# malcolmgreaves/deequ

Measured on AMD Instinct MI355X. Metric: rows/sec (whole node) for fused 16-col profile scan; % of HBM peak BW, higher is better.
Workload: dtype f64+int64+utf8; 1 GPU; C5 fused 16-col profile scan (8 f64 + 4 i64 + 4 utf8, 10% nulls) + state merge + incremental StateLoader append; rows_per_gpu=1000000000, chunk_rows=125000000, analyzers=93, parallelism=row-shard x1

## Files before the change

### deequ_amd/_lib.py

```python
from __future__ import annotations

import ctypes
import os

ABI_VERSION = 6

_HERE = os.path.dirname(os.path.abspath(__file__))
LIB_PATH = os.environ.get("DQ_LIB_PATH") or os.path.join(_HERE, "libdqscan.so")

DQ_OK = 0
DQ_E_INVALID = -1
DQ_E_TYPE = -2
DQ_E_UNSUPPORTED = -3
DQ_E_HIP = -4
DQ_E_OOM = -5
DQ_E_STATE = -6

TYPE_F64, TYPE_I64, TYPE_I32, TYPE_UTF8, TYPE_LARGE_UTF8 = 1, 2, 3, 4, 5
TYPE_F32, TYPE_I16, TYPE_I8, TYPE_BOOL, TYPE_DATE32, TYPE_TIMESTAMP = 6, 7, 8, 9, 10, 11
TYPE_DECIMAL128 = 12


def decimal_type(precision: int, scale: int) -> int:
    if not (1 <= precision <= 38 and 0 <= scale <= precision):
        raise ValueError(f"DecimalType({precision},{scale}) is not a GPU column type (precision 1..38, scale 0..p)")
    return TYPE_DECIMAL128 | precision << 8 | scale << 16

VARIANT_NAMES = {0: "validity", 1: "f64_stats", 2: "f64_stats_hll", 3: "f64_hll", 4: "i64_stats",
                 5: "i64_stats_hll", 6: "i64_hll", 7: "i32_stats", 8: "i32_stats_hll", 9: "i32_hll",
                 10: "utf8_hll", 11: "large_utf8_hll", 12: "utf8_dtype", 13: "utf8_hll_dtype",
                 14: "large_utf8_dtype", 15: "large_utf8_hll_dtype", 16: "f64_dtype",
                 17: "f32_stats", 18: "f32_stats_hll", 19: "f32_hll", 20: "i16_stats", 21: "i16_stats_hll",
                 22: "i16_hll", 23: "i8_stats", 24: "i8_stats_hll", 25: "i8_hll", 26: "f32_dtype", 27: "bool",
                 28: "d128_stats", 29: "d128_stats_hll", 30: "d128_hll", 31: "d128_dtype"}

OP_SIZE = 1
OP_COMPLETENESS = 2
OP_COMPLIANCE = 3
OP_SUM = 4
OP_MEAN = 5
OP_STDDEV = 6
OP_MIN = 7
OP_MAX = 8
OP_CORRELATION = 9
OP_APPROX_COUNT_DISTINCT = 10
OP_DATATYPE = 11
OP_PATTERN_MATCH = 12

PRED_COLUMN = 1
PRED_LIT_INT = 2
PRED_LIT_DECIMAL = 3
PRED_LIT_DOUBLE = 4
PRED_LIT_NULL = 5
PRED_LIT_BOOL = 6
PRED_CMP = 7
PRED_AND = 8
PRED_OR = 9
PRED_NOT = 10
PRED_IS_NULL = 11
PRED_IS_NOT_NULL = 12
PRED_COALESCE = 13
PRED_REGEX = 14

REGEX_RLIKE = 0
REGEX_EXTRACT_NONEMPTY = 1
REGEX_FULL = 2

CMP_LT, CMP_LE, CMP_GT, CMP_GE, CMP_EQ, CMP_NE = 1, 2, 3, 4, 5, 6


class ColumnDesc(ctypes.Structure):
    _fields_ = [("type", ctypes.c_int32), ("nullable", ctypes.c_int32)]


class AnalyzerSpec(ctypes.Structure):
    _fields_ = [("op", ctypes.c_int32), ("col_a", ctypes.c_int32), ("col_b", ctypes.c_int32),
                ("pred_root", ctypes.c_int32), ("where_root", ctypes.c_int32)]


class PredNode(ctypes.Structure):
    _fields_ = [("kind", ctypes.c_int32), ("a", ctypes.c_int32), ("b", ctypes.c_int32),
                ("cmp", ctypes.c_int32), ("i64", ctypes.c_int64), ("f64", ctypes.c_double)]


PRED_PASS = {"auto": 0, "interpreter": 1, "compiled": 2}


class PlanOptions(ctypes.Structure):
    _fields_ = [("struct_size", ctypes.c_int32), ("pred_pass", ctypes.c_int32), ("reserved", ctypes.c_int32 * 6)]


class ColumnView(ctypes.Structure):
    _fields_ = [("values", ctypes.c_void_p), ("validity", ctypes.c_void_p), ("offsets", ctypes.c_void_p),
                ("reserved", ctypes.c_int64)]


class _Size(ctypes.Structure):
    _fields_ = [("num_matches", ctypes.c_int64)]


class _Ratio(ctypes.Structure):
    _fields_ = [("num_matches", ctypes.c_int64), ("count", ctypes.c_int64)]


class _Sum(ctypes.Structure):
    _fields_ = [("sum", ctypes.c_double), ("partial", ctypes.c_int64), ("partial_hi", ctypes.c_int64),
                ("guard", ctypes.c_double), ("dec_scale", ctypes.c_int32), ("dec_digits", ctypes.c_int32)]


class _Mean(ctypes.Structure):
    _fields_ = [("sum", ctypes.c_double), ("count", ctypes.c_int64), ("partial", ctypes.c_int64),
                ("partial_hi", ctypes.c_int64), ("guard", ctypes.c_double), ("dec_scale", ctypes.c_int32),
                ("dec_digits", ctypes.c_int32)]


class _StdDev(ctypes.Structure):
    _fields_ = [("n", ctypes.c_double), ("avg", ctypes.c_double), ("m2", ctypes.c_double)]


class _MinMax(ctypes.Structure):
    _fields_ = [("value", ctypes.c_double)]


class _Corr(ctypes.Structure):
    _fields_ = [("n", ctypes.c_double), ("x_avg", ctypes.c_double), ("y_avg", ctypes.c_double),
                ("ck", ctypes.c_double), ("x_mk", ctypes.c_double), ("y_mk", ctypes.c_double)]


class _Hll(ctypes.Structure):
    _fields_ = [("words", ctypes.c_int64 * 52)]


class _DType(ctypes.Structure):
    _fields_ = [("num_null", ctypes.c_int64), ("num_fractional", ctypes.c_int64), ("num_integral", ctypes.c_int64),
                ("num_boolean", ctypes.c_int64), ("num_string", ctypes.c_int64)]


class _StateUnion(ctypes.Union):
    _fields_ = [("size", _Size), ("ratio", _Ratio), ("sum", _Sum), ("mean", _Mean), ("stddev", _StdDev),
                ("minmax", _MinMax), ("corr", _Corr), ("hll", _Hll), ("dtype", _DType)]


class FreqSummary(ctypes.Structure):
    _fields_ = [("num_groups", ctypes.c_int64), ("num_unique", ctypes.c_int64), ("num_values", ctypes.c_int64),
                ("entropy", ctypes.c_double)]


class State(ctypes.Structure):
    _fields_ = [("op", ctypes.c_int32), ("has_value", ctypes.c_uint8 * 2), ("integral", ctypes.c_uint8),
                ("reserved", ctypes.c_uint8), ("u", _StateUnion)]


STATE_SIZE = ctypes.sizeof(State)


class DQError(RuntimeError):
    def __init__(self, status: int, message: str):
        super().__init__(f"dqscan error {status}: {message}")
        self.status = status
        self.message = message


def _load():
    if not os.path.exists(LIB_PATH):
        raise ImportError(
            f"{LIB_PATH} is missing: build it with `make -C deequ_amd` or __graft_entry__.build(); "
            "the MI355X scan has no CPU fallback")
    import torch
    L = ctypes.CDLL(LIB_PATH)
    c = ctypes
    P = c.POINTER
    L.dq_abi_version.restype = c.c_int32
    L.dq_last_error.restype = c.c_char_p
    L.dq_plan_create.restype = c.c_int32
    L.dq_plan_create.argtypes = [P(AnalyzerSpec), c.c_int32, P(ColumnDesc), c.c_int32, P(PredNode), c.c_int32,
                                 c.c_int32, P(c.c_void_p)]
    L.dq_plan_create_ex.restype = c.c_int32
    L.dq_plan_create_ex.argtypes = [P(AnalyzerSpec), c.c_int32, P(ColumnDesc), c.c_int32, P(PredNode), c.c_int32,
                                    P(c.c_char_p), c.c_int32, c.c_int32, P(c.c_void_p)]
    L.dq_plan_create_opts.restype = c.c_int32
    L.dq_plan_create_opts.argtypes = [P(AnalyzerSpec), c.c_int32, P(ColumnDesc), c.c_int32, P(PredNode), c.c_int32,
                                      P(c.c_char_p), c.c_int32, P(PlanOptions), c.c_int32, P(c.c_void_p)]
    L.dq_plan_explain.restype = c.c_int64
    L.dq_plan_explain.argtypes = [P(AnalyzerSpec), c.c_int32, P(ColumnDesc), c.c_int32, P(PredNode), c.c_int32,
                                  P(c.c_char_p), c.c_int32, P(PlanOptions), c.c_char_p, c.c_int64]
    L.dq_plan_create_time.restype = c.c_int32
    L.dq_plan_create_time.argtypes = [c.c_void_p, P(c.c_double), P(c.c_double)]
    L.dq_regex_info.restype = c.c_int32
    L.dq_regex_info.argtypes = [c.c_char_p, c.c_int32, P(c.c_int32), P(c.c_int32)]
    L.dq_pred_pool_create.restype = c.c_int32
    L.dq_pred_pool_create.argtypes = [P(c.c_char_p), P(c.c_int32), c.c_int32, P(c.c_void_p)]
    L.dq_pred_pool_add.restype = c.c_int32
    L.dq_pred_pool_add.argtypes = [c.c_void_p, c.c_char_p, P(c.c_int32)]
    L.dq_pred_pool_add_regex.restype = c.c_int32
    L.dq_pred_pool_add_regex.argtypes = [c.c_void_p, c.c_int32, c.c_char_p, c.c_int32, P(c.c_int32)]
    L.dq_pred_pool_size.restype = c.c_int32
    L.dq_pred_pool_size.argtypes = [c.c_void_p]
    L.dq_pred_pool_nodes.restype = P(PredNode)
    L.dq_pred_pool_nodes.argtypes = [c.c_void_p]
    L.dq_pred_pool_num_patterns.restype = c.c_int32
    L.dq_pred_pool_num_patterns.argtypes = [c.c_void_p]
    L.dq_pred_pool_patterns.restype = P(c.c_char_p)
    L.dq_pred_pool_patterns.argtypes = [c.c_void_p]
    L.dq_pred_pool_destroy.restype = None
    L.dq_pred_pool_destroy.argtypes = [c.c_void_p]
    L.dq_regex_match_host.restype = c.c_int32
    L.dq_regex_match_host.argtypes = [c.c_char_p, c.c_int32, c.c_void_p, c.c_void_p, c.c_int64, c.c_void_p]
    L.dq_freq_build.restype = c.c_int32
    L.dq_freq_build.argtypes = [P(c.c_int32), c.c_int32, P(ColumnView), P(c.c_int64), c.c_int32, c.c_int32,
                                c.c_void_p, P(c.c_void_p)]
    L.dq_freq_merge.restype = c.c_int32
    L.dq_freq_merge.argtypes = [c.c_void_p, c.c_void_p, P(c.c_void_p)]
    L.dq_freq_summarize.restype = c.c_int32
    L.dq_freq_summarize.argtypes = [c.c_void_p, c.c_int64, P(FreqSummary)]
    L.dq_freq_num_groups.restype = c.c_int64
    L.dq_freq_num_groups.argtypes = [c.c_void_p]
    L.dq_freq_export.restype = c.c_int32
    L.dq_freq_export.argtypes = [c.c_void_p, c.c_void_p, c.c_void_p, c.c_int64]
    L.dq_mutual_information.restype = c.c_int32
    L.dq_mutual_information.argtypes = [P(c.c_int32), P(ColumnView), P(c.c_int64), c.c_int32, c.c_int64, c.c_int32,
                                        c.c_void_p, P(c.c_double), P(c.c_int32)]
    L.dq_approx_quantiles.restype = c.c_int32
    L.dq_approx_quantiles.argtypes = [c.c_int32, P(ColumnView), P(c.c_int64), c.c_int32, P(c.c_double), c.c_int32,
                                      c.c_double, c.c_int32, c.c_void_p, P(c.c_double), P(c.c_int64)]
    L.dq_quantile_digest.restype = c.c_int32
    L.dq_quantile_digest.argtypes = [c.c_int32, P(ColumnView), P(c.c_int64), c.c_int32, c.c_double, c.c_int32,
                                     c.c_void_p, P(c.c_double), P(c.c_int64), c.c_int64, P(c.c_int64), P(c.c_int64)]
    L.dq_freq_top.restype = c.c_int32
    L.dq_freq_top.argtypes = [c.c_void_p, c.c_int32, P(c.c_uint64), P(c.c_int64), P(c.c_uint64), P(c.c_int32)]
    L.dq_freq_destroy.restype = None
    L.dq_freq_destroy.argtypes = [c.c_void_p]
    L.dq_plan_set_stream.restype = c.c_int32
    L.dq_plan_set_stream.argtypes = [c.c_void_p, c.c_void_p]
    L.dq_scan.restype = c.c_int32
    L.dq_scan.argtypes = [c.c_void_p, P(ColumnView), c.c_int64, c.c_int64]
    L.dq_finish.restype = c.c_int32
    L.dq_finish.argtypes = [c.c_void_p, P(State)]
    L.dq_plan_reset.restype = c.c_int32
    L.dq_plan_reset.argtypes = [c.c_void_p]
    L.dq_plan_destroy.restype = None
    L.dq_plan_destroy.argtypes = [c.c_void_p]
    L.dq_plan_bytes_per_row_x1000.restype = c.c_int64
    L.dq_plan_bytes_per_row_x1000.argtypes = [c.c_void_p]
    L.dq_plan_num_launches.restype = c.c_int32
    L.dq_plan_num_launches.argtypes = [c.c_void_p]
    L.dq_plan_enable_timing.restype = c.c_int32
    L.dq_plan_enable_timing.argtypes = [c.c_void_p, c.c_int32]
    L.dq_plan_kernel_time.restype = c.c_int32
    L.dq_plan_kernel_time.argtypes = [c.c_void_p, c.c_int32, P(c.c_double), P(c.c_int64)]
    L.dq_plan_variant_bytes_per_row_x1000.restype = c.c_int64
    L.dq_plan_variant_bytes_per_row_x1000.argtypes = [c.c_void_p, c.c_int32]
    L.dq_plan_kernel_bytes_per_row_x1000.restype = c.c_int64
    L.dq_plan_kernel_bytes_per_row_x1000.argtypes = [c.c_void_p, c.c_int32]
    L.dq_plan_pred_compiled.restype = c.c_int32
    L.dq_plan_pred_compiled.argtypes = [c.c_void_p, c.c_char_p, c.c_int32]
    L.dq_plan_pred_wait.restype = c.c_int32
    L.dq_plan_pred_wait.argtypes = [c.c_void_p, c.c_int32]
    L.dq_state_merge.restype = c.c_int32
    L.dq_state_merge.argtypes = [P(State), P(State), P(State)]
    L.dq_state_combine.restype = c.c_int32
    L.dq_state_combine.argtypes = [P(State), P(State), P(State)]
    for fn in ("dq_state_merge_n", "dq_state_combine_n"):
        getattr(L, fn).restype = c.c_int32
        getattr(L, fn).argtypes = [P(State), P(State), c.c_int32, P(State)]
    L.dq_state_is_defined.restype = c.c_int32
    L.dq_state_is_defined.argtypes = [P(State)]
    L.dq_state_metric.restype = c.c_int32
    L.dq_state_metric.argtypes = [P(State), P(c.c_double)]
    L.dq_hll_estimate.restype = c.c_int32
    L.dq_hll_estimate.argtypes = [P(c.c_int64), P(c.c_double)]
    L.dq_state_to_bytes.restype = c.c_int64
    L.dq_state_to_bytes.argtypes = [P(State), c.c_void_p, c.c_int64]
    L.dq_state_from_bytes.restype = c.c_int32
    L.dq_state_from_bytes.argtypes = [c.c_int32, c.c_char_p, c.c_int64, P(State)]
    L.dq_state_identifier.restype = c.c_int32
    L.dq_state_identifier.argtypes = [c.c_char_p]
    if L.dq_abi_version() != ABI_VERSION:
        raise ImportError(f"libdqscan ABI {L.dq_abi_version()} != {ABI_VERSION}")
    return L


lib = _load()

EXPORTED = [
    "dq_abi_version", "dq_last_error", "dq_plan_create", "dq_plan_create_ex", "dq_plan_create_opts",
    "dq_plan_create_time", "dq_plan_explain", "dq_regex_info", "dq_regex_match_host",
    "dq_pred_pool_create", "dq_pred_pool_add", "dq_pred_pool_add_regex", "dq_pred_pool_size", "dq_pred_pool_nodes",
    "dq_pred_pool_num_patterns", "dq_pred_pool_patterns", "dq_pred_pool_destroy",
    "dq_arrow_import", "dq_uploader_create", "dq_upload", "dq_upload_fence", "dq_upload_release", "dq_upload_sync",
    "dq_uploader_destroy",
    "dq_plan_set_stream", "dq_freq_build", "dq_freq_merge", "dq_freq_summarize", "dq_freq_num_groups",
    "dq_freq_export", "dq_freq_destroy", "dq_mutual_information", "dq_approx_quantiles", "dq_quantile_digest", "dq_freq_top", "dq_scan", "dq_finish",
    "dq_plan_reset", "dq_plan_destroy", "dq_plan_bytes_per_row_x1000", "dq_plan_num_launches",
    "dq_plan_enable_timing", "dq_plan_kernel_time", "dq_plan_variant_bytes_per_row_x1000",
    "dq_plan_kernel_bytes_per_row_x1000", "dq_plan_pred_compiled", "dq_plan_pred_wait",
    "dq_state_merge", "dq_state_combine", "dq_state_merge_n", "dq_state_combine_n", "dq_state_is_defined", "dq_state_metric", "dq_hll_estimate",
    "dq_state_to_bytes", "dq_state_from_bytes", "dq_state_identifier",
]


def check(status: int) -> None:
    if status != DQ_OK:
        raise DQError(status, lib.dq_last_error().decode("utf-8", "replace"))
```

### deequ_amd/csrc/dq_device.h

```cpp
#pragma once

#include <cstdint>

namespace dq {

constexpr int kBlock = 256;
constexpr int kWaves = kBlock / 64;
constexpr int kRowsPerLane = 8;
constexpr int kRowsPerIter = kBlock * kRowsPerLane;
constexpr int kMaxWG = 4096;
constexpr int kTargetWGs = 8192;
constexpr int kMaxCols = 64;
constexpr int kMaxColTasks = 256;
constexpr int kMaxSchemaCols = 1 << 16;
constexpr int kMaxWhere = 8;
constexpr int kHllCopies = 8;
constexpr int kPredAccCopies = 16;
constexpr int kMaxRoots = 32;
constexpr int kMaxCounters = 32;
constexpr int kMaxInstr = 96;
constexpr int kPredStack = 16;
constexpr int kMaxRegexWords = 32768;

enum ColKind : int32_t {
  CK_F64 = 1, CK_I64 = 2, CK_I32 = 3, CK_UTF8 = 4, CK_LUTF8 = 5,
  CK_F32 = 6, CK_I16 = 7, CK_I8 = 8, CK_BOOL = 9,
  CK_D128 = 10,
  CK_D128_LO = 11, CK_D128_HI = 12, CK_D128_LOU = 13,
};
constexpr bool ck_float(int k) { return k == CK_F64 || k == CK_F32; }
constexpr int ck_bytes(int k) {
  return k >= CK_D128 ? 16 : k == CK_F64 || k == CK_I64 ? 8 : k == CK_I32 || k == CK_F32 ? 4 : k == CK_I16 ? 2 : 1;
}

enum ColVariant : int32_t {
  CV_VALIDITY = 0,
  CV_F64_S = 1, CV_F64_SH = 2, CV_F64_H = 3,
  CV_I64_S = 4, CV_I64_SH = 5, CV_I64_H = 6,
  CV_I32_S = 7, CV_I32_SH = 8, CV_I32_H = 9,
  CV_UTF8_H = 10, CV_LUTF8_H = 11,
  CV_UTF8_D = 12, CV_UTF8_HD = 13, CV_LUTF8_D = 14, CV_LUTF8_HD = 15, CV_F64_D = 16,
  CV_F32_S = 17, CV_F32_SH = 18, CV_F32_H = 19,
  CV_I16_S = 20, CV_I16_SH = 21, CV_I16_H = 22,
  CV_I8_S = 23, CV_I8_SH = 24, CV_I8_H = 25,
  CV_F32_D = 26, CV_BOOL = 27,
  CV_D128_S = 28, CV_D128_SH = 29, CV_D128_H = 30, CV_D128_D = 31,
};
constexpr int kNumVariants = 32;

constexpr int kMaxFinRanges = 2 * kNumVariants + 1;
struct FinRanges {
  int32_t n;
  int32_t first[kMaxFinRanges], end[kMaxFinRanges], nr[kMaxFinRanges];
};

struct ColTask {
  int32_t variant;
  int32_t col;
  int32_t where;
  int32_t hll_slot;
  int32_t arg;
  int32_t pad[3];
};

struct PairTask {
  int32_t col_x, col_y;
  int32_t kind_x, kind_y;
  int32_t where;
  int32_t pad[3];
};

constexpr int kTileCols = 8;
constexpr int kTilePairs = 32;
struct PairGroup {
  int32_t ncols;
  int32_t npairs;
  int32_t first_pair;
  int32_t where;
  int32_t cols[kTileCols];
  int32_t kinds[kTileCols];
  int8_t pi[kTilePairs], pj[kTilePairs];
};

constexpr int kPairWaves = 2;
constexpr int kPairPos = 8;
constexpr int kPairSlots = 14;
constexpr int kPairMoments = 4;
constexpr int kPairSlotA[kPairSlots] = {0, 2, 4, 6, 0, 2, 4, 6, 0, 2, 4, 6, 0, 2};
constexpr int kPairSlotB[kPairSlots] = {1, 3, 5, 7, 2, 4, 6, 0, 3, 5, 7, 1, 4, 6};
struct PairWaveTask {
  int32_t where;
  uint32_t pair_mask;
  uint32_t mom_mask;
  uint32_t swap_mask;
  int32_t cols[kPairPos];
  int32_t kinds[kPairPos];
  int32_t pair_out[kPairSlots];
  int32_t mom_out[kPairMoments];
};
struct PairWG {
  PairWaveTask wave[kPairWaves];
};

struct alignas(16) ColPartial {
  double n, mean, m2;
  double sum;
  int64_t isum;
  int64_t count;
  int64_t nan_count;
  double fmin, fmax;
  int64_t pinf_count;
  int64_t ninf_count;
  int64_t isum_hi;
};
static_assert(sizeof(ColPartial) == 96, "ColPartial layout");

struct alignas(16) CorrPartial {
  double n, xa, ya, ck, xm, ym, pad0, pad1;
};
static_assert(sizeof(CorrPartial) == 64, "CorrPartial layout");

struct alignas(16) PredPartial {
  int64_t t[kMaxCounters];
  int64_t nn[kMaxCounters];
};

enum PredOp : int32_t {
  PO_ATOM_CMP = 1,
  PO_ATOM_ISNULL = 2,
  PO_ATOM_NOTNULL = 3,
  PO_CONST = 4,
  PO_AND = 5,
  PO_OR = 6,
  PO_NOT = 7,
  PO_STORE = 8,
  PO_ATOM_REGEX = 9,
};
enum CmpOp : int32_t { C_LT = 1, C_LE = 2, C_GT = 3, C_GE = 4, C_EQ = 5, C_NE = 6, C_FALSE = 7, C_TRUE = 8 };
enum CmpType : int32_t { CT_INT = 1, CT_DBL = 2 };
enum NullRes : int32_t { NR_FALSE = 0, NR_TRUE = 1, NR_NULL = 2 };

struct PredInstr {
  int32_t op;
  int32_t cmp;
  int32_t ctype;
  int32_t null_res;
  int32_t col_a;
  int32_t col_b;
  int32_t kind_a;
  int32_t kind_b;
  int64_t lit_i;
  double lit_d;
  int32_t slot;
  int32_t pad;
};

struct PredCounter {
  int32_t pred;
  int32_t where;
};

struct PredProgram {
  const uint16_t* regex;
  int32_t regex_words;
  int32_t n_instr;
  int32_t n_counters;
  int32_t n_bitmaps;
  int32_t n_loads;
  int32_t n_roots;
  int32_t stack_depth;
  int16_t load_instr[kMaxInstr];
  int32_t bitmap_root[kMaxWhere];
  PredCounter counters[kMaxCounters];
  PredInstr instr[kMaxInstr];
};

struct ScanCols {
  const void* values[kMaxCols];
  const uint32_t* validity[kMaxCols];
  const void* offsets[kMaxCols];
};

struct ScanBitmaps {
  uint64_t* where_bits[kMaxWhere];
  int64_t* rare_rows;
};

}
```

### deequ_amd/csrc/dq_kernels.hip

```cpp
#include <hip/hip_runtime.h>

#include <cstdint>
#include <type_traits>

#include "dq_device.h"
#include "dq_hash.h"
#include "dq_decimal.h"
#include "dq_lane.h"

namespace dq {

#define DQ_DEC_TABLE static __constant__ const
#include "dq_dec_tables.inc"
#undef DQ_DEC_TABLE
__device__ __forceinline__ DecTab dec_dev_tab() { return DecTab{kDecP10Lo, kDecP10Hi, kDecRcpHi, kDecRcpLo}; }

typedef uint32_t u32x4 __attribute__((ext_vector_type(4)));

__device__ __forceinline__ uint32_t ld32(const uint8_t* base, int64_t a) {
  return *reinterpret_cast<const uint32_t*>(base + a);
}
__device__ __forceinline__ uint32_t read4(const uint8_t* base, int64_t pos) {
  int64_t a = pos & ~int64_t(3);
  uint32_t sh = (uint32_t)(pos & 3) * 8u;
// ... 262 lines not shown
      const bool two = r + 32 < row1;
      if (validity) sel = ((uint64_t)(two ? ((const_u32s)validity)[w + 1] : 0u) << 32) | ((const_u32s)validity)[w];
      if (mask) sel &= ((uint64_t)(two ? ((const_u32s)mask)[w + 1] : 0u) << 32) | ((const_u32s)mask)[w];
      if (r + 64 > row1) sel &= (1ull << (row1 - r)) - 1ull;
    }
    if (sel == 0) continue;
    const double x = range_value<KIND>(vr, r - row0 + lane);
    const uint64_t fm = __builtin_amdgcn_ballot_w64(__builtin_isfinite(x)) & sel;
    if (fm != 0) return wave_uniform(wave_sum_f64(lane_bit(fm) ? x : 0.0) / (double)__builtin_popcountll(fm));
  }
  return 0.0;
}

template <bool INTEGRAL, bool MINMAX_SEP>
__device__ __forceinline__ void masked_moments(LaneMoments& a, double& lo, double& hi, double x, uint64_t b,
                                               double shift, uint64_t ma, uint64_t mb) {
  double d;
  uint64_t save;
  if constexpr (INTEGRAL) {
    asm volatile(
        "s_and_saveexec_b64 %[save], %[ma]\n\t"
        "v_add_f64 %[d], %[x], -%[sh]\n\t"
        "v_lshl_add_u64 %[is], %[b], 0, %[is]\n\t"
        "v_min_f64 %[lo], %[lo], %[x]\n\t"
        "v_max_f64 %[hi], %[hi], %[x]\n\t"
        "v_add_f64 %[sd], %[sd], %[d]\n\t"
        "v_fma_f64 %[sdd], %[d], %[d], %[sdd]\n\t"
        "s_mov_b64 exec, %[save]"
        : [sd] "+v"(a.sd), [sdd] "+v"(a.sdd), [is] "+v"(a.is), [lo] "+v"(lo), [hi] "+v"(hi), [d] "=&v"(d),
          [save] "=&s"(save)
        : [x] "v"(x), [sh] "s"(shift), [b] "v"(b), [ma] "s"(ma)
        : "scc");
  } else if constexpr (!MINMAX_SEP) {
    asm volatile(
        "s_and_saveexec_b64 %[save], %[ma]\n\t"
        "v_add_f64 %[d], %[x], -%[sh]\n\t"
        "v_min_f64 %[lo], %[lo], %[x]\n\t"
        "v_max_f64 %[hi], %[hi], %[x]\n\t"
        "v_add_f64 %[sd], %[sd], %[d]\n\t"
        "v_fma_f64 %[sdd], %[d], %[d], %[sdd]\n\t"
        "s_mov_b64 exec, %[save]"
        : [sd] "+v"(a.sd), [sdd] "+v"(a.sdd), [lo] "+v"(lo), [hi] "+v"(hi), [d] "=&v"(d), [save] "=&s"(save)
        : [x] "v"(x), [sh] "s"(shift), [ma] "s"(ma)
        : "scc");
  } else {
    asm volatile(
        "s_and_saveexec_b64 %[save], %[ma]\n\t"
        "v_add_f64 %[d], %[x], -%[sh]\n\t"
        "v_add_f64 %[sd], %[sd], %[d]\n\t"
        "v_fma_f64 %[sdd], %[d], %[d], %[sdd]\n\t"
        "s_and_b64 exec, %[save], %[mb]\n\t"
        "v_min_f64 %[lo], %[lo], %[x]\n\t"
        "v_max_f64 %[hi], %[hi], %[x]\n\t"
        "s_mov_b64 exec, %[save]"
        : [sd] "+v"(a.sd), [sdd] "+v"(a.sdd), [lo] "+v"(lo), [hi] "+v"(hi), [d] "=&v"(d), [save] "=&s"(save)
        : [x] "v"(x), [sh] "s"(shift), [ma] "s"(ma), [mb] "s"(mb)
        : "scc");
  }
}

template <int KIND, bool STATS, bool HLL>
__device__ __forceinline__ void numeric_block(const double (&x)[8], const uint64_t (&bits)[8], const uint64_t (&m)[8],
                                              double shift, ColStats& s, LaneMoments& a, int32_t* regs, int32_t& qmin) {
#pragma unroll
  for (int j = 0; j < 8; ++j) {
    if (STATS) masked_moments<!ck_float(KIND), false>(a, s.fmin, s.fmax, x[j], bits[j], shift, m[j], m[j]);
    if (HLL) {
      const HllKey key = ck_bytes(KIND) <= 4 ? hll_key_int((uint32_t)bits[j]) : hll_key_long(bits[j]);
      qmin = min(qmin, key.q);
      if (lane_bit(m[j])) atomicMax(reinterpret_cast<int32_t*>(reinterpret_cast<char*>(regs) + key.addr), key.q);
    }
  }
  if (HLL) {
    if (__builtin_amdgcn_ballot_w64(qmin < 0) != 0) {
#pragma unroll 1
      for (int j = 0; j < 8; ++j) {
        if (lane_bit(m[j])) hll_update(regs, ck_bytes(KIND) <= 4 ? xxh64_int((uint32_t)bits[j]) : xxh64_long(bits[j]));
      }
      qmin = 0;
    }
  }
}

template <int KIND, bool STATS, bool HLL>
__device__ __forceinline__ void float_block_checked(__amdgpu_buffer_rsrc_t vr, const uint32_t* validity,
                                                    const uint32_t* mask, int64_t base, int32_t rem, int32_t vo,
                                                    double shift, ColStats& s, LaneMoments& a, int32_t* regs,
                                                    int64_t& cnt_w, int64_t& nan_v, int64_t& pinf_v, int64_t& ninf_v) {
  constexpr bool kF32 = KIND == CK_F32;
  const int lane = threadIdx.x & 63;
#pragma unroll 1
  for (int j = 0; j < 8; ++j) {
    const int32_t left = rem - 64 * j;
    if (left <= 0) break;
    const int64_t r = base + 64 * j;
    uint64_t mj = ~0ull;
    {
      const int64_t w = r >> 5;
      const bool two = left > 32;
      if (validity) mj = ((uint64_t)(two ? ((const_u32s)validity)[w + 1] : 0u) << 32) | ((const_u32s)validity)[w];
      if (mask) mj &= ((uint64_t)(two ? ((const_u32s)mask)[w + 1] : 0u) << 32) | ((const_u32s)mask)[w];
      if (left < 64) mj &= (1ull << left) - 1ull;
    }
    uint64_t b;
    double xv;
    if constexpr (kF32) {
      b = __builtin_amdgcn_raw_buffer_load_b32(vr, vo + j * 256, 0, 2 );
      xv = (double)__builtin_bit_cast(float, (uint32_t)b);
    } else {
      const auto w2 = __builtin_amdgcn_raw_buffer_load_b64(vr, vo + j * 512, 0, 2 );
      b = ((uint64_t)w2[1] << 32) | w2[0];
      xv = __builtin_bit_cast(double, b);
    }
    const uint64_t nf = __builtin_amdgcn_ballot_w64(!__builtin_isfinite(xv)) & mj;
    const uint64_t nanm = __builtin_amdgcn_ballot_w64(xv != xv) & mj;
    const uint64_t inf = nf & ~nanm, pinf = __builtin_amdgcn_ballot_w64(xv > 0.0) & inf;
    if (lane == 0) {
      nan_v += __builtin_popcountll(nanm);
      pinf_v += __builtin_popcountll(pinf);
      ninf_v += __builtin_popcountll(inf & ~pinf);
    }
    if (STATS) {
      const uint64_t mm = mj & ~inf;
      cnt_w += __builtin_popcountll(mm);
      masked_moments<false, true>(a, s.fmin, s.fmax, xv, b, shift, mm, mj & ~nanm);
    } else {
      cnt_w += __builtin_popcountll(mj);
    }
    if (HLL) {
      if (lane_bit(nanm)) b = kF32 ? 0x7FC00000ull : 0x7FF8000000000000ull;
      const HllKey key = kF32 ? hll_key_int((uint32_t)b) : hll_key_long(b);
      if (lane_bit(mj)) {
        if (key.q >= 0) atomicMax(reinterpret_cast<int32_t*>(reinterpret_cast<char*>(regs) + key.addr), key.q);
        else hll_update(regs, kF32 ? xxh64_int((uint32_t)b) : xxh64_long(b));
      }
    }
  }
}

template <int K> struct KindT { using T = double; };
template <> struct KindT<CK_I64> { using T = int64_t; };
template <> struct KindT<CK_I32> { using T = int32_t; };
template <> struct KindT<CK_F32> { using T = float; };
template <> struct KindT<CK_I16> { using T = int16_t; };
template <> struct KindT<CK_I8> { using T = int8_t; };

template <int KIND, bool STATS, bool HLL>
__device__ void numeric_range(const void* values, const uint32_t* validity, const uint32_t* mask,
                              int64_t row0, int64_t row1, ColStats& s, int32_t* regs) {
  using T = typename KindT<KIND>::T;
  constexpr bool kLazy = ck_float(KIND) && STATS;
  const int lane = threadIdx.x & 63;
  const int wave = __builtin_amdgcn_readfirstlane(threadIdx.x >> 6);
  const T* v = reinterpret_cast<const T*>(values);
  const __amdgpu_buffer_rsrc_t vr = __builtin_amdgcn_make_buffer_rsrc(
      const_cast<T*>(v + row0), (short)0, (int)((row1 - row0) * (int64_t)sizeof(T)), 0x00020000);
  int64_t nan_v = 0, pinf_v = 0, ninf_v = 0;
  int64_t cnt_w = 0;
  LaneMoments a{0.0, 0.0, 0};
  const double shift = STATS ? range_shift_of<KIND>(vr, validity, mask, row0, row1, lane) : 0.0;
  int32_t qmin = 0;
  const int32_t nr = (int32_t)(row1 - row0);
  for (int32_t rb = 0; rb < nr; rb += kRowsPerIter) {
    const int64_t base = row0 + rb + wave * 512;
    const int32_t rem = nr - rb - wave * 512;
    const bool full = rb + kRowsPerIter <= nr;
    uint64_t bits[8], m[8];
    double x[8];
    const int32_t vo = (rb + wave * 512 + lane) * (int32_t)sizeof(T);
#pragma unroll
    for (int j = 0; j < 8; ++j) {
      if constexpr (sizeof(T) == 8) {
        const auto w2 = __builtin_amdgcn_raw_buffer_load_b64(vr, vo + j * 512, 0, 2 );
        bits[j] = ((uint64_t)w2[1] << 32) | w2[0];
        if (KIND == CK_F64) x[j] = __builtin_bit_cast(double, bits[j]);
        else x[j] = __builtin_fma((double)(int32_t)w2[1], 4294967296.0, (double)w2[0]);
      } else if constexpr (KIND == CK_F32) {
        const uint32_t w = __builtin_amdgcn_raw_buffer_load_b32(vr, vo + j * 256, 0, 2 );
        bits[j] = w;
        x[j] = (double)__builtin_bit_cast(float, w);
      } else {
        int32_t w;
        if constexpr (sizeof(T) == 4) w = (int32_t)__builtin_amdgcn_raw_buffer_load_b32(vr, vo + j * 256, 0, 2 );
        else if constexpr (sizeof(T) == 2) w = (int16_t)__builtin_amdgcn_raw_buffer_load_b16(vr, vo + j * 128, 0, 2 );
        else w = (int8_t)__builtin_amdgcn_raw_buffer_load_b8(vr, vo + j * 64, 0, 2 );
        bits[j] = (uint64_t)(int64_t)w;
        x[j] = (double)w;
      }
    }
    block_masks(validity, mask, base, rem, full, m);
    uint64_t nf_any = 0;
    if constexpr (ck_float(KIND) && !kLazy) {
#pragma unroll
      for (int j = 0; j < 8; ++j) nf_any |= __builtin_amdgcn_ballot_w64(!__builtin_isfinite(x[j])) & m[j];
    }
    if (ck_float(KIND) && !kLazy && nf_any != 0) {
      float_block_checked<KIND, STATS, HLL>(vr, validity, mask, base, rem, vo, shift, s, a, regs, cnt_w, nan_v, pinf_v,
                                            ninf_v);
    } else {
#pragma unroll
      for (int j = 0; j < 8; ++j) cnt_w += __builtin_popcountll(m[j]);
      numeric_block<KIND, STATS, HLL>(x, bits, m, shift, s, a, regs, qmin);
    }
  }
  if constexpr (kLazy) {
    __shared__ int32_t redo;
    if (threadIdx.x == 0) redo = 0;
    __syncthreads();
    const bool bad = !__builtin_isfinite(a.sd) || !__builtin_isfinite(a.sdd);
    if (__builtin_amdgcn_ballot_w64(bad) != 0 && lane == 0) redo = 1;
    __syncthreads();
    if (redo) {
      if (HLL) {
        for (int i = threadIdx.x; i < 512; i += kBlock) regs[i] = -1;
      }
      stats_init(s);
      a = LaneMoments{0.0, 0.0, 0};
      cnt_w = 0;
      __syncthreads();
      for (int32_t rb = 0; rb < nr; rb += kRowsPerIter) {
        const int32_t vo = (rb + wave * 512 + lane) * (int32_t)sizeof(T);
        float_block_checked<KIND, STATS, HLL>(vr, validity, mask, row0 + rb + wave * 512, nr - rb - wave * 512, vo,
                                              shift, s, a, regs, cnt_w, nan_v, pinf_v, ninf_v);
      }
    }
  }
  if (STATS) {
    const double S1 = wave_sum_f64(a.sd), S2 = wave_sum_f64(a.sdd);
    const int64_t is = ck_float(KIND) ? 0 : wave_sum_i64(a.is);
    if (lane == 0 && cnt_w > 0) {
      const double n = (double)cnt_w, q = S1 / n;
      s.n = n;
      s.mean = shift + q;
      const double m2 = __builtin_fma(-S1, q, S2);
      s.m2 = m2 < 0.0 ? 0.0 : m2;
      if (ck_float(KIND)) s.sum = __builtin_fma(n, shift, S1);
      else s.isum = is;
    }
  }
  if (lane == 0) s.count += cnt_w;
  if (ck_float(KIND) && lane == 0) {
    s.nan_count += nan_v;
    s.pinf += pinf_v;
    s.ninf += ninf_v;
    if (STATS) s.count += pinf_v + ninf_v;
  }
}

enum DtClass : uint32_t { DT_FRACTIONAL = 1, DT_INTEGRAL = 2, DT_BOOLEAN = 3, DT_STRING = 4 };

__device__ __forceinline__ uint32_t dt_class_of(bool numeric, uint32_t dots, bool boolean) {
  return numeric && dots <= 1 ? (dots ? DT_FRACTIONAL : DT_INTEGRAL) : (boolean ? DT_BOOLEAN : DT_STRING);
}

__device__ __forceinline__ uint32_t dt_keep(int lo, int hi) {
  const uint32_t below_hi = hi >= 4 ? 0x80808080u : (hi <= 0 ? 0u : 0x80808080u & ((1u << (8 * hi)) - 1u));
  const uint32_t from_lo = lo <= 0 ? 0x80808080u : (lo >= 4 ? 0u : 0x80808080u & ~((1u << (8 * lo)) - 1u));
  return below_hi & from_lo;
}

__device__ __forceinline__ uint32_t dt_class_short(const uint32_t (&w)[8], uint32_t len, bool active) {
  const uint32_t b0 = w[0] & 0xFFu;
  const uint32_t sgn = (len > 0 && (b0 == 0x2Bu || b0 == 0x2Du)) ? 1u : 0u;
  const uint32_t start = sgn + ((sgn < len && ((w[0] >> (8 * sgn)) & 0xFFu) == 0x20u) ? 1u : 0u);
  uint32_t bad = 0, dots = 0;
#pragma unroll
  for (int k = 0; k < 7; ++k) {
    if (k > 0 && __builtin_amdgcn_ballot_w64(active && bad == 0 && dots <= 1 && (uint32_t)(4 * k) < len) == 0) break;
    const uint32_t keep = dt_keep((int)start - 4 * k, (int)len - 4 * k);
    const uint32_t t = w[k] ^ 0x30303030u, z = w[k] ^ 0x2E2E2E2Eu;
    const uint32_t nd = ((t & 0x7F7F7F7Fu) + 0x76767676u) | t;
    const uint32_t nz = ((z & 0x7F7F7F7Fu) + 0x7F7F7F7Fu) | z;
    bad |= nd & nz & keep;
    dots += __builtin_popcount(~nz & keep);
  }
  const bool boolean = (len == 4 && w[0] == 0x65757274u) ||
                       (len == 5 && w[0] == 0x736C6166u && (w[1] & 0xFFu) == 0x65u);
  return dt_class_of(bad == 0, dots, boolean);
}

__device__ uint32_t dt_class_bytes(const uint8_t* p, int64_t len) {
  int64_t i = 0;
  if (len > 0 && (p[0] == '+' || p[0] == '-')) i = 1;
  if (i < len && p[i] == ' ') ++i;
  bool numeric = true;
  uint32_t dots = 0;
// ... 476 lines not shown
  const int32_t nr = (int32_t)(row1 - row0);
  for (int32_t rb = 0; rb < nr; rb += kRowsPerIter) {
    const int64_t base = row0 + rb + wave * 512;
    const int32_t rem = nr - rb - wave * 512;
    uint64_t m[8];
    block_masks(validity, mask, base, rem, rb + kRowsPerIter <= nr, m);
    uint64_t lo[8], hi[8];
#pragma unroll
    for (int j = 0; j < 8; ++j) load(base + 64 * j + lane, lo[j], hi[j]);
#pragma unroll
    for (int j = 0; j < 8; ++j) {
      cnt_w += __builtin_popcountll(m[j]);
      const bool sel = lane_bit(m[j]);
      if constexpr (STATS) {
        const double x = dec_to_double(lo[j], hi[j], sc, tab, prec <= 18);
        masked_moments<false, false>(a, s.fmin, s.fmax, x, 0, shift, m[j], m[j]);
        if (sel) {
          const uint64_t l2 = slo + lo[j];
          shi += hi[j] + (l2 < slo ? 1u : 0u);
          slo = l2;
          guard += x;
        }
      }
      if constexpr (HLL) {
        const uint64_t b = dec_hash_head(lo[j], hi[j], prec);
        const HllKey key = hll_key_from_fmix(b);
        if (sel) {
          if (key.q >= 0) atomicMax(reinterpret_cast<int32_t*>(reinterpret_cast<char*>(regs) + key.addr), key.q);
          else hll_update(regs, fmix_tail(b));
        }
      }
      if constexpr (DT) frac += __builtin_popcountll(__builtin_amdgcn_ballot_w64(dec_dt_class(lo[j], hi[j], sc, tab) == 1) & m[j]);
    }
  }
  if constexpr (STATS) {
    const double S1 = wave_sum_f64(a.sd), S2 = wave_sum_f64(a.sdd), G = wave_sum_f64(guard);
#pragma unroll
    for (int k = 32; k >= 1; k >>= 1) {
      const uint64_t olo = __shfl_xor(slo, k), ohi = __shfl_xor(shi, k);
      const uint64_t l2 = slo + olo;
      shi = shi + ohi + (l2 < slo ? 1u : 0u);
      slo = l2;
    }
    if (lane == 0 && cnt_w > 0) {
      const double n = (double)cnt_w, q = S1 / n;
      s.n = n;
      s.mean = shift + q;
      const double m2 = __builtin_fma(-S1, q, S2);
      s.m2 = m2 < 0.0 ? 0.0 : m2;
      s.sum = G;
      s.isum = (int64_t)slo;
      s.isum_hi = (int64_t)shi;
    }
  }
  if (lane == 0) {
    s.count += cnt_w;
    if (DT) s.isum += frac;
  }
}

__device__ void validity_range(const uint32_t* validity, const uint32_t* mask, int64_t row0, int64_t row1, ColStats& s) {
  const int64_t w0 = row0 >> 5, w1 = (row1 + 31) >> 5;
  int64_t c = 0;
  for (int64_t w = w0 + threadIdx.x; w < w1; w += kBlock) {
    uint32_t bits = word_or_ones(validity, w);
    if (mask) bits &= mask[w];
    const int64_t r = w << 5;
    if (r + 32 > row1) bits &= (1u << (row1 - r)) - 1u;
    c += __popc(bits);
  }
  s.count += c;
}

template <int KIND, bool STATS, bool HLL>
__device__ void run_numeric(const ColTask& t, const ScanCols& cols, const ScanBitmaps& bm, int64_t row0, int64_t row1,
                            ColStats& s, int32_t* regs) {
  const uint32_t* mask = t.where >= 0 ? reinterpret_cast<const uint32_t*>(bm.where_bits[t.where]) : nullptr;
  numeric_range<KIND, STATS, HLL>(cols.values[t.col], cols.validity[t.col], mask, row0, row1, s, regs);
}

template <int V, bool LONG>
__device__ __forceinline__ void run_variant(const ColTask& t, const ScanCols& cols, const uint32_t* mask, int64_t row0,
                                            int64_t row1, int64_t n_rows, ColStats& s, int32_t* regs,
                                            const uint64_t* p5, uint32_t* dq, uint32_t* rare, uint32_t* cls) {
  const void* v = cols.values[t.col];
  const uint32_t* val = cols.validity[t.col];
  if constexpr (V == CV_VALIDITY) validity_range(val, mask, row0, row1, s);
  else if constexpr (V == CV_F64_S) numeric_range<CK_F64, true, false>(v, val, mask, row0, row1, s, regs);
  else if constexpr (V == CV_F64_SH) numeric_range<CK_F64, true, true>(v, val, mask, row0, row1, s, regs);
  else if constexpr (V == CV_F64_H) numeric_range<CK_F64, false, true>(v, val, mask, row0, row1, s, regs);
  else if constexpr (V == CV_I64_S) numeric_range<CK_I64, true, false>(v, val, mask, row0, row1, s, regs);
  else if constexpr (V == CV_I64_SH) numeric_range<CK_I64, true, true>(v, val, mask, row0, row1, s, regs);
  else if constexpr (V == CV_I64_H) numeric_range<CK_I64, false, true>(v, val, mask, row0, row1, s, regs);
  else if constexpr (V == CV_I32_S) numeric_range<CK_I32, true, false>(v, val, mask, row0, row1, s, regs);
  else if constexpr (V == CV_I32_SH) numeric_range<CK_I32, true, true>(v, val, mask, row0, row1, s, regs);
  else if constexpr (V == CV_I32_H) numeric_range<CK_I32, false, true>(v, val, mask, row0, row1, s, regs);
  else if constexpr (V == CV_F32_S) numeric_range<CK_F32, true, false>(v, val, mask, row0, row1, s, regs);
  else if constexpr (V == CV_F32_SH) numeric_range<CK_F32, true, true>(v, val, mask, row0, row1, s, regs);
  else if constexpr (V == CV_F32_H) numeric_range<CK_F32, false, true>(v, val, mask, row0, row1, s, regs);
  else if constexpr (V == CV_I16_S) numeric_range<CK_I16, true, false>(v, val, mask, row0, row1, s, regs);
  else if constexpr (V == CV_I16_SH) numeric_range<CK_I16, true, true>(v, val, mask, row0, row1, s, regs);
  else if constexpr (V == CV_I16_H) numeric_range<CK_I16, false, true>(v, val, mask, row0, row1, s, regs);
  else if constexpr (V == CV_I8_S) numeric_range<CK_I8, true, false>(v, val, mask, row0, row1, s, regs);
  else if constexpr (V == CV_I8_SH) numeric_range<CK_I8, true, true>(v, val, mask, row0, row1, s, regs);
  else if constexpr (V == CV_I8_H) numeric_range<CK_I8, false, true>(v, val, mask, row0, row1, s, regs);
  else if constexpr (V == CV_F64_D) float_dtype_range(reinterpret_cast<const double*>(v), val, mask, row0, row1, s);
  else if constexpr (V == CV_F32_D) float_dtype_range(reinterpret_cast<const float*>(v), val, mask, row0, row1, s);
  else if constexpr (V == CV_BOOL) bool_range(reinterpret_cast<const uint32_t*>(v), val, mask, row0, row1, s, regs);
  else if constexpr (V == CV_D128_S) decimal_range<true, false, false>(v, val, mask, row0, row1, s, regs, t.arg);
  else if constexpr (V == CV_D128_SH) decimal_range<true, true, false>(v, val, mask, row0, row1, s, regs, t.arg);
  else if constexpr (V == CV_D128_H) decimal_range<false, true, false>(v, val, mask, row0, row1, s, regs, t.arg);
  else if constexpr (V == CV_D128_D) decimal_range<false, false, true>(v, val, mask, row0, row1, s, regs, t.arg);
  else if constexpr (V == CV_UTF8_H || V == CV_UTF8_D || V == CV_UTF8_HD)
    utf8_range<int32_t, V != CV_UTF8_D, V != CV_UTF8_H, LONG>(
        reinterpret_cast<const uint8_t*>(v), reinterpret_cast<const int32_t*>(cols.offsets[t.col]), val, mask, row0,
        row1, n_rows, s, regs, p5, dq, rare, cls);
  else
    utf8_range<int64_t, V != CV_LUTF8_D, V != CV_LUTF8_H, LONG>(
        reinterpret_cast<const uint8_t*>(v), reinterpret_cast<const int64_t*>(cols.offsets[t.col]), val, mask, row0,
        row1, n_rows, s, regs, p5, dq, rare, cls);
}

#ifndef DQ_STR_WAVES
#define DQ_STR_WAVES 6
#endif
#ifndef DQ_NUM_WAVES
#define DQ_NUM_WAVES 6
#endif
template <int V, bool LONG>
constexpr int kMinWaves = V == CV_UTF8_H && !LONG && DQ_STR_CLS ? 5
                          : V == CV_UTF8_H && DQ_STR_WAVES > 0 ? DQ_STR_WAVES
                          : (V == CV_F64_SH || V == CV_I64_SH) && DQ_NUM_WAVES > 0 ? DQ_NUM_WAVES
                          : V == CV_LUTF8_H && LONG ? 5
                                                    : 1;

template <int V, bool LONG = false>
__global__ __launch_bounds__(kBlock) __attribute__((amdgpu_waves_per_eu(kMinWaves<V, LONG>))) void dq_column_scan(const ColTask* __restrict__ tasks, int32_t ntasks,
                                                         int32_t part_base, ScanCols cols, ScanBitmaps bm,
                                                         int64_t n_rows, int64_t rows_per_range,
                                                         ColPartial* __restrict__ partials,
                                                         uint32_t* __restrict__ hll_acc) {
  constexpr bool kHll = !(V == CV_VALIDITY || V == CV_F64_S || V == CV_I64_S || V == CV_I32_S || V == CV_F64_D ||
                         V == CV_UTF8_D || V == CV_LUTF8_D || V == CV_F32_S || V == CV_I16_S || V == CV_I8_S ||
                         V == CV_F32_D || V == CV_BOOL || V == CV_D128_S || V == CV_D128_D);
  constexpr bool kBool = V == CV_BOOL;
  constexpr bool kStr = V == CV_UTF8_H || V == CV_LUTF8_H || V == CV_UTF8_HD || V == CV_LUTF8_HD;
  __shared__ int32_t regs[kHll ? 512 : 2];
  __shared__ uint64_t p5[kStr ? 256 : 1];
  constexpr uint32_t kDCap = DQ_STR_CLS && (V == CV_UTF8_H || V == CV_LUTF8_H) && !LONG ? kDefCapCls : kDefCap;
  __shared__ uint32_t dfq[kStr ? kWaves * kDefFields * kDCap : 1];
  __shared__ uint32_t rare[kStr ? kWaves : 1];
  constexpr bool kCls = DQ_STR_CLS && (V == CV_UTF8_H || V == CV_LUTF8_H) && !LONG;
  __shared__ __attribute__((aligned(16))) uint32_t clsbuf[kCls ? kWaves * kClsWords : 4];
  __shared__ ColStats red[kWaves];
  const int32_t ti = blockIdx.x % ntasks;
  const int32_t range = blockIdx.x / ntasks;
  const ColTask t = tasks[ti];
  const int64_t row0 = (int64_t)range * rows_per_range;
  int64_t row1 = row0 + rows_per_range;
  if (row1 > n_rows) row1 = n_rows;
  if constexpr (kBool) {
    if (threadIdx.x < 2) regs[threadIdx.x] = 0;
    __syncthreads();
  }
  if constexpr (kHll) {
    for (int i = threadIdx.x; i < 512; i += kBlock) regs[i] = -1;
    if constexpr (kStr) {
      p5[threadIdx.x] = (uint64_t)threadIdx.x * XP5;
      if (threadIdx.x < kWaves) rare[threadIdx.x] = 0;
    }
    __syncthreads();
  }
  ColStats s;
  stats_init(s);
  const uint32_t* mask = t.where >= 0 ? reinterpret_cast<const uint32_t*>(bm.where_bits[t.where]) : nullptr;
  const int32_t wv = kStr ? __builtin_amdgcn_readfirstlane(threadIdx.x >> 6) : 0;
  run_variant<V, LONG>(t, cols, mask, row0, row1, n_rows, s, regs, p5, dfq + wv * kDefFields * kDCap, rare + wv,
                       clsbuf + (kCls ? wv * kClsWords : 0));
  block_reduce_store(s, partials + (size_t)(part_base + ti) * kMaxWG + range, red);
  if constexpr (kStr) {
    if (threadIdx.x == 0 && bm.rare_rows) {
      uint32_t r = 0;
      for (int w = 0; w < kWaves; ++w) r += rare[w];
      if (r) atomicAdd(reinterpret_cast<unsigned long long*>(bm.rare_rows + part_base + ti), (unsigned long long)r);
    }
  }
  if constexpr (kBool) {
    if (threadIdx.x == 0 && t.hll_slot >= 0) {
      uint32_t* dst = hll_acc + ((size_t)t.hll_slot * kHllCopies + (blockIdx.x % kHllCopies)) * 512;
      for (int b = 0; b < 2; ++b) {
        if (!regs[b]) continue;
        const uint64_t x = xxh64_int(b == 0 ? 1u : 0u);
        atomicMax(dst + (uint32_t)(x >> 55), (uint32_t)(hll_q_exact(x) + 1));
      }
    }
  }
  if constexpr (kHll) {
    __syncthreads();
    uint32_t* dst = hll_acc + ((size_t)t.hll_slot * kHllCopies + (blockIdx.x % kHllCopies)) * 512;
    for (int i = threadIdx.x; i < 512; i += kBlock) {
      const uint32_t v = (uint32_t)(regs[i] + 1);
      if (v > __builtin_nontemporal_load(dst + i)) atomicMax(dst + i, v);
    }
  }
}

struct CorrStats { double n, xa, ya, ck, xm, ym; };

__device__ __forceinline__ void corr_merge(CorrStats& a, const CorrStats& b) {
  double n = a.n + b.n;
  if (b.n != 0.0) {
    if (a.n == 0.0) { a.xa = b.xa; a.ya = b.ya; a.ck = b.ck; a.xm = b.xm; a.ym = b.ym; }
    else {
      double dx = b.xa - a.xa, dy = b.ya - a.ya;
      double r = b.n / n;
      double dxr = dx * r, dyr = dy * r;
      a.ck = a.ck + b.ck + dx * dyr * a.n;
      a.xm = a.xm + b.xm + dx * dxr * a.n;
      a.ym = a.ym + b.ym + dy * dyr * a.n;
      a.xa = a.xa + dxr;
      a.ya = a.ya + dyr;
    }
  }
  a.n = n;
}

__device__ __forceinline__ int cmp_dbl(double a, double b) {
  bool an = a != a, bn = b != b;
  if (an || bn) return (an && bn) ? 0 : (an ? 1 : -1);
  return (a > b) - (a < b);
}
__device__ __forceinline__ bool apply_cmp(int op, int c) {
  switch (op) {
    case C_LT: return c < 0;
    case C_LE: return c <= 0;
    case C_GT: return c > 0;
    case C_GE: return c >= 0;
    case C_EQ: return c == 0;
    case C_NE: return c != 0;
    case C_TRUE: return true;
    default: return false;
  }
}

struct PredScratch {
  uint32_t *st, *sn, *rt, *rn, *ct, *cn;
  __device__ PredScratch(uint32_t* w, int depth, int roots, int counters) {
    st = w; sn = st + 16 * depth; rt = sn + 16 * depth; rn = rt + 16 * roots; ct = rn + 16 * roots; cn = ct + 16 * counters;
  }
};

__device__ __forceinline__ void pred_load(const void* p, int kind, int64_t row0, int64_t row1, int64_t base, int lane,
                                          uint64_t (&v)[8]) {
  if (kind == CK_BOOL) {
    const __amdgpu_buffer_rsrc_t r = __builtin_amdgcn_make_buffer_rsrc(
        const_cast<char*>(reinterpret_cast<const char*>(p) + (row0 >> 3)), (short)0, (int)(((row1 - row0 + 31) >> 5) * 4),
        0x00020000);
#pragma unroll
    for (int j = 0; j < 8; ++j) {
      const uint32_t w = __builtin_amdgcn_raw_buffer_load_b32(r, (int)(((base - row0) >> 5) + 2 * j + (lane >> 5)) * 4, 0, 0);
      v[j] = (w >> (lane & 31)) & 1u;
    }
    return;
  }
  const int sz = ck_bytes(kind);
  const __amdgpu_buffer_rsrc_t r = __builtin_amdgcn_make_buffer_rsrc(
      const_cast<char*>(reinterpret_cast<const char*>(p) + row0 * sz), (short)0, (int)((row1 - row0) * sz), 0x00020000);
  if (kind == CK_I32) {
#pragma unroll
    for (int j = 0; j < 8; ++j)
      v[j] = (uint64_t)(int64_t)(int32_t)__builtin_amdgcn_raw_buffer_load_b32(r, lane * 4, (int)((base - row0 + 64 * j) * 4), 2);
  } else if (kind == CK_F32) {
#pragma unroll
    for (int j = 0; j < 8; ++j)
      v[j] = __builtin_bit_cast(uint64_t, (double)__builtin_bit_cast(
                                              float, __builtin_amdgcn_raw_buffer_load_b32(r, (int)((base - row0 + 64 * j + lane) * 4), 0, 2)));
  } else if (kind == CK_I16) {
#pragma unroll
    for (int j = 0; j < 8; ++j)
      v[j] = (uint64_t)(int64_t)(int16_t)__builtin_amdgcn_raw_buffer_load_b16(r, (int)((base - row0 + 64 * j + lane) * 2), 0, 2);
  } else if (kind == CK_I8) {
#pragma unroll
    for (int j = 0; j < 8; ++j)
      v[j] = (uint64_t)(int64_t)(int8_t)__builtin_amdgcn_raw_buffer_load_b8(r, (int)(base - row0 + 64 * j + lane), 0, 2);
  } else if (kind >= CK_D128_LO) {
// ... 345 lines not shown
          for (int j = 0; j < 8; ++j) dst[j] = C.a[j];
        }
        vdst = C.va;
      } else if (same_blk && col == C.t_col_b && C.t_vals && (!vals || kind == C.t_kind_b)) {
        if (vals) {
#pragma unroll
          for (int j = 0; j < 8; ++j) dst[j] = C.b[j];
        }
        vdst = C.vb;
      } else {
        if (vals) pred_load(cols.values[col], kind, row0, row1, base, lane, dst);
        vdst = pred_valid_word(cols.validity[col], base, n_rows, lane);
      }
    };
    const bool cmp = op == PO_ATOM_CMP;
    if (cmp && col_b >= 0) fetch(col_b, kind_b, true, L.b, L.vb);
    fetch(col_a, kind_a, cmp, L.a, L.va);
    L.t_base = base;
    L.t_col_a = col_a;
    L.t_col_b = cmp ? col_b : -1;
    L.t_kind_a = kind_a;
    L.t_kind_b = kind_b;
    L.t_vals = cmp;
  };
  if (n_loads > 0) issue(0, row0 + (int64_t)wave * 512, B0, B1);
  uint32_t g = 0;

  for (int64_t blk = row0; blk < row1; blk += kRowsPerIter) {
    const int64_t base = blk + (int64_t)wave * 512;
    if (base >= row1) break;
    const int64_t wr = base + 32 * (lane & 15);
    const uint32_t inr = wr >= row1 ? 0u : (wr + 32 <= row1 ? ~0u : ((1u << (row1 - wr)) - 1u));
    int sp = 0, k = 0;
    for (int i = 0; i < n_instr; ++i) {
      const uint32_t ow = __builtin_amdgcn_readfirstlane(s_op[i]);
      const int op = (int)(ow & 0xFFu);
      if (op == PO_ATOM_CMP || op == PO_ATOM_ISNULL || op == PO_ATOM_NOTNULL || op == PO_ATOM_REGEX) {
        const int kn = k + 1 < n_loads ? k + 1 : 0;
        const int64_t bn = k + 1 < n_loads ? base : base + kRowsPerIter;
        uint32_t wt, wn;
        const AtomBuf& cur = (g & 1u) ? B1 : B0;
        if ((g & 1u) == 0) issue(kn, bn, B1, B0);
        else issue(kn, bn, B0, B1);
        if (op == PO_ATOM_CMP) {
          const PredInstr ins = uniform_cmp_fields(&s_instr[i]);
          if ((g & 1u) == 0) pred_atom_cmp(ins, B0, lane, wt, wn);
          else pred_atom_cmp(ins, B1, lane, wt, wn);
        } else if (RX && op == PO_ATOM_REGEX) {
          const PredInstr ins = uniform_instr(&s_instr[i]);
          const uint32_t va = (g & 1u) ? B1.va : B0.va;
          if (ins.kind_a == CK_UTF8)
            pred_atom_regex_utf8(ins, dfa_lds + ins.lit_i, reinterpret_cast<const uint8_t*>(cols.values[ins.col_a]),
                                 reinterpret_cast<const int32_t*>(cols.offsets[ins.col_a]), n_rows, row1, base, lane,
                                 va, wt, wn);
          else
            pred_atom_regex(ins, dfa_lds + ins.lit_i, reinterpret_cast<const uint8_t*>(cols.values[ins.col_a]),
                            cols.offsets[ins.col_a], row1, base, lane, va, wt, wn);
        } else {
          const uint32_t va = (g & 1u) ? B1.va : B0.va;
          wt = op == PO_ATOM_ISNULL ? ~va : va;
          wn = 0u;
        }
        (void)cur;
        ++g;
        ++k;
        if (wl) { S.st[(sp) * 16 + lane] = wt; S.sn[(sp) * 16 + lane] = wn; }
        ++sp;
      } else {
        pred_logic_op(ow, S, sp, lane);
      }
    }
    pred_block_out(S, s_ctr, n_counters, s_bmroot, n_bitmaps, bm, wr, inr, n_rows, lane);
  }
  pred_counters_out(pred_lds, wave_words, prog, acc);
}

__global__ __launch_bounds__(kBlock) void dq_finalize(int32_t ncol, int32_t nranges_col,
                                                      const ColPartial* __restrict__ col_part,
                                                      ColPartial* __restrict__ col_acc, int32_t npair, int32_t nranges_pair,
                                                      const CorrPartial* __restrict__ pair_part,
                                                      CorrPartial* __restrict__ pair_acc, int32_t has_pred,
                                                      int32_t nranges_pred, const PredPartial* __restrict__ pred_part,
                                                      PredPartial* __restrict__ pred_acc, FinRanges fr,
                                                      int64_t* __restrict__ rare_dev, int64_t* rare_host) {
  __shared__ ColStats cs[kBlock];
  __shared__ CorrStats ps[kBlock];
  const int b = blockIdx.x, tid = threadIdx.x;
  if (b < ncol) {
    int32_t nr = nranges_col;
    for (int i = 0; i < fr.n; ++i)
      if (b >= fr.first[i] && b < fr.end[i]) nr = fr.nr[i];
    ColStats s;
    stats_init(s);
    for (int r = tid; r < nr; r += kBlock) stats_merge(s, stats_load(col_part + (size_t)b * kMaxWG + r));
    cs[tid] = s;
    __syncthreads();
    for (int stride = kBlock / 2; stride >= 1; stride >>= 1) {
      if (tid < stride) { ColStats a = cs[tid]; stats_merge(a, cs[tid + stride]); cs[tid] = a; }
      __syncthreads();
    }
    if (tid == 0) {
      ColStats acc = stats_load(col_acc + b);
      stats_merge(acc, cs[0]);
      stats_store(col_acc + b, acc);
      if (rare_host && rare_dev[b] != rare_dev[ncol + b]) {
        rare_dev[ncol + b] = rare_dev[b];
        __hip_atomic_store(rare_host + b, rare_dev[b], __ATOMIC_RELAXED, __HIP_MEMORY_SCOPE_SYSTEM);
      }
    }
  } else if (b < ncol + npair) {
    const int p = b - ncol;
    CorrStats s = {0, 0, 0, 0, 0, 0};
    for (int r = tid; r < nranges_pair; r += kBlock) {
      const CorrPartial& q = pair_part[(size_t)p * kMaxWG + r];
      CorrStats o = {q.n, q.xa, q.ya, q.ck, q.xm, q.ym};
      corr_merge(s, o);
    }
    ps[tid] = s;
    __syncthreads();
    for (int stride = kBlock / 2; stride >= 1; stride >>= 1) {
      if (tid < stride) { CorrStats a = ps[tid]; corr_merge(a, ps[tid + stride]); ps[tid] = a; }
      __syncthreads();
    }
    if (tid == 0) {
      CorrPartial& q = pair_acc[p];
      CorrStats acc = {q.n, q.xa, q.ya, q.ck, q.xm, q.ym};
      corr_merge(acc, ps[0]);
      q.n = acc.n; q.xa = acc.xa; q.ya = acc.ya; q.ck = acc.ck; q.xm = acc.xm; q.ym = acc.ym;
    }
  } else if (has_pred) {
    static_assert(kBlock % kMaxCounters == 0, "counter layout");
    constexpr int G = kBlock / kMaxCounters;
    __shared__ int64_t st[G][kMaxCounters], sn[G][kMaxCounters];
    const int c = tid % kMaxCounters, g = tid / kMaxCounters;
    int64_t t = 0, nn = 0;
    for (int r = g; r < nranges_pred; r += G) { t += pred_part[r].t[c]; nn += pred_part[r].nn[c]; }
    st[g][c] = t;
    sn[g][c] = nn;
    __syncthreads();
    if (tid < kMaxCounters) {
      int64_t a = pred_acc->t[tid], b = pred_acc->nn[tid];
      for (int k = 0; k < G; ++k) { a += st[k][tid]; b += sn[k][tid]; }
      pred_acc->t[tid] = a;
      pred_acc->nn[tid] = b;
    }
  }
}

__global__ void dq_init_acc(ColPartial* col_acc, int32_t ncol, CorrPartial* pair_acc, int32_t npair, int64_t* rare_dev) {
  const int i = blockIdx.x * blockDim.x + threadIdx.x;
  if (i < ncol) {
    ColStats s;
    stats_init(s);
    stats_store(col_acc + i, s);
    if (rare_dev) rare_dev[i] = 0;
  }
  if (i < npair) {
    CorrPartial& q = pair_acc[i];
    q.n = q.xa = q.ya = q.ck = q.xm = q.ym = q.pad0 = q.pad1 = 0.0;
  }
}

hipError_t launch_pred_scan(const PredProgram* prog, const ScanCols& cols, const ScanBitmaps& bm, int64_t n_rows,
                            int64_t rows_per_range, int32_t nranges, PredPartial* acc, int32_t lds_bytes, hipStream_t st,
                            bool has_regex) {
  if (has_regex)
    hipLaunchKernelGGL(dq_pred_scan<true>, dim3(nranges), dim3(kBlock), (size_t)lds_bytes, st, prog, cols, bm, n_rows,
                       rows_per_range, acc);
  else
    hipLaunchKernelGGL(dq_pred_scan<false>, dim3(nranges), dim3(kBlock), (size_t)lds_bytes, st, prog, cols, bm, n_rows,
                       rows_per_range, acc);
  return hipGetLastError();
}

template <int V>
static void launch_v(const ColTask* tasks, int32_t ntasks, int32_t part_base, const ScanCols& cols,
                     const ScanBitmaps& bm, int64_t n_rows, int64_t rows_per_range, int32_t nranges,
                     ColPartial* partials, uint32_t* hll_acc, bool long_str, hipStream_t st) {
  constexpr bool kStrHll = V == CV_UTF8_H || V == CV_LUTF8_H || V == CV_UTF8_HD || V == CV_LUTF8_HD;
  if constexpr (kStrHll) {
    if (long_str) {
      hipLaunchKernelGGL((dq_column_scan<V, true>), dim3((uint32_t)ntasks * (uint32_t)nranges), dim3(kBlock), 0, st,
                         tasks, ntasks, part_base, cols, bm, n_rows, rows_per_range, partials, hll_acc);
      return;
    }
  }
  hipLaunchKernelGGL(dq_column_scan<V>, dim3((uint32_t)ntasks * (uint32_t)nranges), dim3(kBlock), 0, st, tasks, ntasks,
                     part_base, cols, bm, n_rows, rows_per_range, partials, hll_acc);
}

hipError_t launch_column_scan(int32_t variant, const ColTask* tasks, int32_t ntasks, int32_t part_base,
                              const ScanCols& cols, const ScanBitmaps& bm, int64_t n_rows, int64_t rows_per_range,
                              int32_t nranges, ColPartial* partials, uint32_t* hll_acc, bool long_str, hipStream_t st) {
#define DQ_V(V)                                                                                            \
  case V:                                                                                                  \
    launch_v<V>(tasks, ntasks, part_base, cols, bm, n_rows, rows_per_range, nranges, partials, hll_acc, long_str, \
                st);                                                                                       \
    break;
  switch (variant) {
    DQ_V(CV_VALIDITY) DQ_V(CV_F64_S) DQ_V(CV_F64_SH) DQ_V(CV_F64_H) DQ_V(CV_I64_S) DQ_V(CV_I64_SH) DQ_V(CV_I64_H)
    DQ_V(CV_I32_S) DQ_V(CV_I32_SH) DQ_V(CV_I32_H) DQ_V(CV_UTF8_H) DQ_V(CV_LUTF8_H)
    DQ_V(CV_UTF8_D) DQ_V(CV_UTF8_HD) DQ_V(CV_LUTF8_D) DQ_V(CV_LUTF8_HD) DQ_V(CV_F64_D)
    DQ_V(CV_F32_S) DQ_V(CV_F32_SH) DQ_V(CV_F32_H) DQ_V(CV_I16_S) DQ_V(CV_I16_SH) DQ_V(CV_I16_H)
    DQ_V(CV_I8_S) DQ_V(CV_I8_SH) DQ_V(CV_I8_H) DQ_V(CV_F32_D) DQ_V(CV_BOOL)
    DQ_V(CV_D128_S) DQ_V(CV_D128_SH) DQ_V(CV_D128_H) DQ_V(CV_D128_D)
    default: return hipErrorInvalidValue;
  }
#undef DQ_V
  return hipGetLastError();
}


hipError_t launch_finalize(int32_t ncol, int32_t nranges_col, const ColPartial* col_part, ColPartial* col_acc,
                           int32_t npair, int32_t nranges_pair, const CorrPartial* pair_part, CorrPartial* pair_acc,
                           int32_t has_pred, int32_t nranges_pred, const PredPartial* pred_part, PredPartial* pred_acc,
                           const FinRanges& fr, int64_t* rare_dev, int64_t* rare_host, hipStream_t st) {
  const uint32_t nb = (uint32_t)(ncol + npair + (has_pred ? 1 : 0));
  if (nb == 0) return hipSuccess;
  hipLaunchKernelGGL(dq_finalize, dim3(nb), dim3(kBlock), 0, st, ncol, nranges_col, col_part, col_acc, npair,
                     nranges_pair, pair_part, pair_acc, has_pred, nranges_pred, pred_part, pred_acc, fr, rare_dev,
                     rare_host);
  return hipGetLastError();
}

hipError_t launch_init_acc(ColPartial* col_acc, int32_t ncol, CorrPartial* pair_acc, int32_t npair, int64_t* rare_dev,
                           hipStream_t st) {
  const int n = ncol > npair ? ncol : npair;
  if (n == 0) return hipSuccess;
  hipLaunchKernelGGL(dq_init_acc, dim3((n + 255) / 256), dim3(256), 0, st, col_acc, ncol, pair_acc, npair, rare_dev);
  return hipGetLastError();
}

}
```

### deequ_amd/csrc/dq_plan.cpp

```cpp
#include <hip/hip_runtime.h>

#include <algorithm>
#include <chrono>
#include <cmath>
#include <cstdarg>
#include <cstdio>
#include <cstdlib>
#include <cstring>
#include <functional>
#include <iterator>
#include <limits>
#include <map>
#include <memory>
#include <string>
#include <tuple>
#include <vector>

#include "dq_device.h"
#include "dq_internal.h"
#include "dq_pred_jit.h"

#ifndef DQ_MIN_RANGE_ROWS
#define DQ_MIN_RANGE_ROWS 16384
#endif
#ifndef DQ_MIN_VALIDITY_RANGE_ROWS
#define DQ_MIN_VALIDITY_RANGE_ROWS 65536
#endif
#ifndef DQ_F64_HLL_DIV
#define DQ_F64_HLL_DIV 2
#endif
#ifndef DQ_PAIR_ONE_ROUND
#define DQ_PAIR_ONE_ROUND 1
#endif
#ifndef DQ_PRED_WGS
#define DQ_PRED_WGS 2048
#endif
#include "dq_regex.h"

namespace dq {

hipError_t launch_pred_scan(const PredProgram* prog, const ScanCols& cols, const ScanBitmaps& bm, int64_t n_rows,
                            int64_t rows_per_range, int32_t nranges, PredPartial* acc, int32_t lds_bytes, hipStream_t st,
                            bool has_regex);
hipError_t launch_column_scan(int32_t variant, const ColTask* tasks, int32_t ntasks, int32_t part_base,
                              const ScanCols& cols, const ScanBitmaps& bm, int64_t n_rows, int64_t rows_per_range,
                              int32_t nranges, ColPartial* partials, uint32_t* hll_acc, bool long_str, hipStream_t st);
hipError_t launch_pair_scan(const PairWG* wgs, int32_t nwg, const ScanCols& cols, const ScanBitmaps& bm,
                            const uint32_t* ones, int64_t n_rows, int64_t rows_per_range, int32_t nranges,
                            CorrPartial* pair_part, ColPartial* col_part, int32_t* redo, bool all_f64, bool ring,
                            bool minmax, hipStream_t st);
hipError_t pair_scan_residency(bool all_f64, bool ring, bool minmax, int32_t* per_cu);
hipError_t launch_finalize(int32_t ncol, int32_t nranges_col, const ColPartial* col_part, ColPartial* col_acc,
                           int32_t npair, int32_t nranges_pair, const CorrPartial* pair_part, CorrPartial* pair_acc,
                           int32_t has_pred, int32_t nranges_pred, const PredPartial* pred_part, PredPartial* pred_acc, const FinRanges& fr, int64_t* rare_dev, int64_t* rare_host,
                           hipStream_t st);
hipError_t launch_init_acc(ColPartial* col_acc, int32_t ncol, CorrPartial* pair_acc, int32_t npair, int64_t* rare_dev,
                           hipStream_t st);

static thread_local char g_err[1024] = "";
static thread_local bool g_capacity = false;

dq_status set_error(dq_status code, const char* fmt, ...) {
  va_list ap;
  va_start(ap, fmt);
  std::vsnprintf(g_err, sizeof(g_err), fmt, ap);
  va_end(ap);
  return code;
}

static dq_status cap_error(const char* fmt, ...) {
  va_list ap;
  va_start(ap, fmt);
  std::vsnprintf(g_err, sizeof(g_err), fmt, ap);
  va_end(ap);
  g_capacity = true;
  return DQ_E_UNSUPPORTED;
}

#define HIP_TRY(expr)                                                                              \
  do {                                                                                             \
    hipError_t e_ = (expr);                                                                        \
    if (e_ != hipSuccess)                                                                          \
      return set_error(e_ == hipErrorOutOfMemory ? DQ_E_OOM : DQ_E_HIP, "%s failed: %s (%s:%d)", \
                       #expr, hipGetErrorString(e_), __FILE__, __LINE__);                          \
  } while (0)

static bool is_numeric(int32_t t) {
  return t == DQ_TYPE_F64 || t == DQ_TYPE_I64 || t == DQ_TYPE_I32 || t == DQ_TYPE_F32 || t == DQ_TYPE_I16 ||
         t == DQ_TYPE_I8 || is_decimal(t);
}
static bool is_integral(int32_t t) { return t == DQ_TYPE_I64 || t == DQ_TYPE_I32 || t == DQ_TYPE_I16 || t == DQ_TYPE_I8; }
static bool is_floating(int32_t t) { return t == DQ_TYPE_F64 || t == DQ_TYPE_F32; }
static bool is_string(int32_t t) { return t == DQ_TYPE_UTF8 || t == DQ_TYPE_LARGE_UTF8; }
static int32_t kind_of(int32_t t) {
  switch (t) {
    case DQ_TYPE_F64: return CK_F64;
    case DQ_TYPE_I64: case DQ_TYPE_TIMESTAMP: return CK_I64;
    case DQ_TYPE_I32: case DQ_TYPE_DATE32: return CK_I32;
    case DQ_TYPE_F32: return CK_F32;
    case DQ_TYPE_I16: return CK_I16;
    case DQ_TYPE_I8: return CK_I8;
    case DQ_TYPE_BOOL: return CK_BOOL;
    case DQ_TYPE_UTF8: return CK_UTF8;
    case DQ_TYPE_LARGE_UTF8: return CK_LUTF8;
    default: return CK_D128;
  }
}
static int32_t pair_kind(int32_t t) {
  if (!is_decimal(t)) return kind_of(t);
  return CK_D128 | DQ_DECIMAL_SCALE(t) << 8 | (DQ_DECIMAL_PRECISION(t) <= 18 ? 1 : 0) << 16;
}
static int64_t value_bytes_x1000(int32_t t) {
  switch (t) {
    case DQ_TYPE_I32: case DQ_TYPE_F32: case DQ_TYPE_DATE32: case DQ_TYPE_UTF8: return 4000;
    case DQ_TYPE_I16: return 2000;
    case DQ_TYPE_I8: return 1000;
    case DQ_TYPE_BOOL: return 125;
    default: return is_decimal(t) ? 16000 : 8000;
  }
}
static double int_as_float(int64_t v) { return (double)(float)v; }

struct SpecOut {
  int32_t op = 0;
  int32_t col_task = -1;
  int32_t pair_task = -1;
  int32_t ctr_a = -1;
  int32_t ctr_b = -1;
  int32_t col_type = 0;
  bool has_where = false;
};

struct Lit {
  enum K { INT, DEC, DBL, NUL, BOOL } k;
  int64_t i = 0;
  int32_t scale = 0;
  double d = 0.0;
};

// ... 401 lines not shown
          return set_error(DQ_E_UNSUPPORTED, "float column compared with an int / long column");
        PredInstr p{};
        p.op = PO_ATOM_CMP; p.col_a = ca; p.col_b = cb; p.kind_a = kind_of(ta); p.kind_b = kind_of(tb);
        p.null_res = NR_NULL; p.cmp = to_cmpop(cmp);
        p.ctype = bools || (is_integral(ta) && is_integral(tb)) ? CT_INT : CT_DBL;
        out.push_back(p);
        return DQ_OK;
      }
      default:
        return set_error(DQ_E_UNSUPPORTED, "predicate node kind %d is not a boolean expression", n.kind);
    }
  }
};

static std::string canon(const dq_pred_node* pool, int32_t n_pred, int32_t idx, int depth = 0) {
  if (idx < 0 || idx >= n_pred || depth > 64) return "?";
  const dq_pred_node& n = pool[idx];
  char buf[128];
  std::snprintf(buf, sizeof(buf), "(%d:%d:%lld:%a", n.kind, n.cmp, (long long)n.i64, n.f64);
  std::string s = buf;
  if (n.kind == DQ_PRED_COLUMN) s += ":c" + std::to_string(n.a);
  else {
    if (n.kind == DQ_PRED_CMP || n.kind == DQ_PRED_AND || n.kind == DQ_PRED_OR || n.kind == DQ_PRED_NOT ||
        n.kind == DQ_PRED_IS_NULL || n.kind == DQ_PRED_IS_NOT_NULL || n.kind == DQ_PRED_COALESCE ||
        n.kind == DQ_PRED_REGEX)
      s += canon(pool, n_pred, n.a, depth + 1);
    if (n.kind == DQ_PRED_CMP || n.kind == DQ_PRED_AND || n.kind == DQ_PRED_OR || n.kind == DQ_PRED_COALESCE)
      s += canon(pool, n_pred, n.b, depth + 1);
  }
  return s + ")";
}

}

using namespace dq;

struct dq_plan {
  int32_t device = 0;
  hipStream_t stream = nullptr;
  bool own_stream = false;
  std::vector<dq_column_desc> schema;
  std::vector<dq_analyzer_spec> specs;
  std::vector<SpecOut> outs;

  std::vector<ColTask> col_tasks;
  struct Group { int32_t variant, first, count; };
  std::vector<Group> groups;
  std::vector<Group> pred_fused_groups;
  std::vector<PairTask> pair_tasks;
  std::vector<PairWG> pair_wgs;
  int32_t n_fused = 0;
  bool pair_all_f64 = true;
  bool pair_minmax = false;
  PredProgram prog{};
  std::vector<std::string> patterns;
  std::vector<uint16_t> regex_blob;
  uint16_t* d_regex = nullptr;
  int32_t n_hll = 0;
  bool has_pred = false;
  hipFunction_t pred_jit = nullptr;
  PredJitRef pred_jit_ref;
  std::vector<int32_t> pred_jit_cols;
  std::vector<int32_t> pred_jit_hll_task, pred_jit_hll_slot;
  int32_t pred_fused_first = 0, pred_fused_count = 0;
  int32_t pair_fused_first = 0, pair_fused_count = 0;
  int32_t pair_resident[2] = {0, 0};
  std::string pred_jit_note;
  int32_t pred_pass = DQ_PRED_PASS_AUTO;
  bool host_only = false;
  bool probe = false;
  std::string pred_jit_src;
  double create_ms = 0.0, pred_jit_ms = 0.0;

  ColTask* d_col_tasks = nullptr;
  PairTask* d_pair_tasks = nullptr;
  PairWG* d_pair_wgs = nullptr;
  int32_t* d_pair_redo = nullptr;
  char* h_stage = nullptr;
  int64_t* d_rare_dev = nullptr;
  int64_t* h_rare = nullptr;
  int64_t* d_rare = nullptr;
  std::vector<uint8_t> str_long;
  int32_t str_path = 0;
  int64_t prev_rows = 0;
  size_t h_stage_bytes = 0;
  PredProgram* d_prog = nullptr;
  ColPartial* d_col_part = nullptr;
  CorrPartial* d_pair_part = nullptr;
  PredPartial* d_pred_part = nullptr;
  ColPartial* d_col_acc = nullptr;
  uint32_t* d_hll_acc = nullptr;
  CorrPartial* d_pair_acc = nullptr;
  PredPartial* d_pred_acc = nullptr;
  uint64_t* d_where_bits[kMaxWhere] = {nullptr};
  int64_t where_cap_words = 0;
  uint32_t* d_ones = nullptr;
  int64_t ones_cap_words = 0;

  int64_t total_rows = 0;
  int64_t next_chunk = 0;

  bool timing = false;
  std::vector<hipEvent_t> ev_pool;
  struct Pending { int kernel; hipEvent_t a, b; };
  std::vector<Pending> pending;
  static constexpr int kTimers = 16 + kNumVariants;
  double kernel_ms[kTimers] = {0};
  int64_t kernel_launches[kTimers] = {0};
  int64_t bytes_per_row_x1000 = 0;
  int64_t pred_bytes_x1000 = 0, pair_bytes_x1000 = 0;
  int32_t launches_per_scan = 0;

  std::vector<dq_plan*> parts;
  std::vector<std::vector<int32_t>> part_specs;
  std::vector<std::vector<int32_t>> part_cols;
};

static dq_status take_event(dq_plan* p, hipEvent_t* e) {
  if (!p->ev_pool.empty()) { *e = p->ev_pool.back(); p->ev_pool.pop_back(); return DQ_OK; }
  HIP_TRY(hipEventCreate(e));
  return DQ_OK;
}

static dq_status resolve_timing(dq_plan* p) {
  if (p->pending.empty()) return DQ_OK;
  HIP_TRY(hipStreamSynchronize(p->stream));
  for (auto& q : p->pending) {
    float ms = 0.f;
    HIP_TRY(hipEventElapsedTime(&ms, q.a, q.b));
    p->kernel_ms[q.kernel] += ms;
    p->kernel_launches[q.kernel] += 1;
    p->ev_pool.push_back(q.a);
    p->ev_pool.push_back(q.b);
  }
  p->pending.clear();
  return DQ_OK;
}

template <typename F>
static dq_status timed(dq_plan* p, int kernel, hipStream_t st, F fn) {
  hipEvent_t a = nullptr, b = nullptr;
  if (p->timing) {
    if (dq_status s = take_event(p, &a)) return s;
    if (dq_status s = take_event(p, &b)) return s;
    HIP_TRY(hipEventRecord(a, st));
  }
  HIP_TRY(fn());
  if (p->timing) {
    HIP_TRY(hipEventRecord(b, st));
    p->pending.push_back({kernel, a, b});
  }
  return DQ_OK;
}

static dq_status free_plan_mem(dq_plan* p) {
  for (auto& q : p->pending) { p->ev_pool.push_back(q.a); p->ev_pool.push_back(q.b); }
  p->pending.clear();
  for (hipEvent_t e : p->ev_pool) (void)hipEventDestroy(e);
  p->ev_pool.clear();
  void* ptrs[] = {p->d_col_tasks, p->d_pair_tasks, p->d_pair_wgs, p->d_prog, p->d_col_part, p->d_pair_part,
                  p->d_pred_part, p->d_col_acc, p->d_hll_acc, p->d_pair_acc, p->d_pred_acc, p->d_regex, p->d_pair_redo,
                  p->d_rare_dev};
  for (void* q : ptrs)
    if (q) (void)hipFree(q);
  for (int i = 0; i < kMaxWhere; ++i)
    if (p->d_where_bits[i]) (void)hipFree(p->d_where_bits[i]);
  if (p->d_ones) (void)hipFree(p->d_ones);
  if (p->h_rare) (void)hipHostFree(p->h_rare);
  p->h_rare = p->d_rare = nullptr;
  if (p->h_stage) (void)hipHostFree(p->h_stage);
  p->h_stage = nullptr;
  p->h_stage_bytes = 0;
  return DQ_OK;
}

static dq_status reset_acc(dq_plan* p) {
  HIP_TRY(launch_init_acc(p->d_col_acc, (int32_t)p->col_tasks.size(), p->d_pair_acc, (int32_t)p->pair_tasks.size(),
                          p->d_rare_dev, p->stream));
  if (p->n_hll) HIP_TRY(hipMemsetAsync(p->d_hll_acc, 0, (size_t)p->n_hll * kHllCopies * 512 * sizeof(uint32_t), p->stream));
  if (p->has_pred) HIP_TRY(hipMemsetAsync(p->d_pred_acc, 0, kPredAccCopies * sizeof(PredPartial), p->stream));
  if (p->total_rows > 0) p->prev_rows = p->total_rows;
  p->total_rows = 0;
  p->next_chunk = 0;
  return DQ_OK;
}

template <typename T>
static dq_status dmalloc(T** ptr, size_t bytes) {
  if (bytes == 0) bytes = 16;
  HIP_TRY(hipMalloc((void**)ptr, bytes));
  return DQ_OK;
}

static void plan_pair_wgs(const dq_plan* p, const PairGroup& g, std::vector<PairWG>& out, std::vector<int>& fused) {
  auto blank = [&](const int32_t* lcols, int nl) {
    PairWG wg;
    std::memset(&wg, 0, sizeof(wg));
    for (int w = 0; w < kPairWaves; ++w) {
      PairWaveTask& t = wg.wave[w];
      t.where = g.where;
      for (int q = 0; q < kPairPos; ++q) {
        const int l = (q + w) % kPairPos;
        const int c = lcols[l < nl ? l : 0];
        t.cols[q] = g.cols[c];
        t.kinds[q] = g.kinds[c];
      }
      for (int q = 0; q < kPairSlots; ++q) t.pair_out[q] = -1;
      for (int k = 0; k < kPairMoments; ++k) t.mom_out[k] = -1;
    }
    return wg;
  };
  auto place = [&](PairWG& wg, int a, int b, int32_t pair) {
    for (int w = 0; w < kPairWaves; ++w) {
      const int pa = (a - w + kPairPos) % kPairPos, pb = (b - w + kPairPos) % kPairPos;
      for (int q = 0; q < kPairSlots; ++q) {
        const bool fwd = kPairSlotA[q] == pa && kPairSlotB[q] == pb, rev = kPairSlotA[q] == pb && kPairSlotB[q] == pa;
        if (!fwd && !rev) continue;
        PairWaveTask& t = wg.wave[w];
        if ((t.pair_mask >> q) & 1u) return false;
        t.pair_mask |= 1u << q;
        if (rev) t.swap_mask |= 1u << q;
        t.pair_out[q] = pair;
        return true;
      }
    }
    return false;
  };
  int32_t ident[kPairPos];
  for (int c = 0; c < kPairPos; ++c) ident[c] = c;
  PairWG wg = blank(ident, g.ncols);
  std::vector<int> extra;
  for (int q = 0; q < g.npairs; ++q)
    if (g.pi[q] == g.pj[q] || !place(wg, g.pi[q], g.pj[q], g.first_pair + q)) extra.push_back(q);
  for (int c = 0; c < g.ncols; ++c)
    for (size_t t = 0; t < p->col_tasks.size(); ++t) {
      const ColTask& ct = p->col_tasks[t];
      if (ct.col == g.cols[c] && ct.where == g.where && !fused[t] &&
          (ct.variant == CV_F64_S || ct.variant == CV_I64_S || ct.variant == CV_I32_S || ct.variant == CV_F32_S ||
           ct.variant == CV_I16_S || ct.variant == CV_I8_S)) {
        PairWaveTask& w = wg.wave[c % 2];
        const int k = (c - c % 2) / 2;
        w.mom_mask |= 1u << k;
        w.mom_out[k] = (int32_t)t;
        fused[t] = 1;
        break;
      }
    }
  if (wg.wave[0].pair_mask | wg.wave[0].mom_mask | wg.wave[1].pair_mask | wg.wave[1].mom_mask) out.push_back(wg);
  for (int q : extra) {
    const int32_t lc[2] = {g.pi[q], g.pj[q]};
    PairWG e = blank(lc, 2);
    PairWaveTask& t = e.wave[0];
    t.pair_mask = 1u;
    t.pair_out[0] = g.first_pair + q;
    out.push_back(e);
  }
}

static dq_status build_plan(dq_plan* p, const dq_pred_node* pool, int32_t n_pred) {
  const int32_t ncols = (int32_t)p->schema.size();
  std::map<std::string, int32_t> root_slot;
// ... 384 lines not shown
      p->pred_fused_groups.back().count++;
    }
    p->n_fused = (int32_t)std::count_if(fused.begin(), fused.end(), [](int f) { return f != 0; });
  }

  std::vector<int> need_values(ncols, 0), need_validity(ncols, 0);
  for (const ColTask& ct : p->col_tasks) {
    need_validity[ct.col] = 1;
    if (ct.variant != CV_VALIDITY) need_values[ct.col] = 1;
  }
  for (const PairTask& pt : p->pair_tasks) {
    need_values[pt.col_x] = need_values[pt.col_y] = 1;
    need_validity[pt.col_x] = need_validity[pt.col_y] = 1;
  }
  for (int i = 0; i < prog.n_instr; ++i) {
    const PredInstr& ins = prog.instr[i];
    if (ins.col_a >= 0) {
      need_validity[ins.col_a] = 1;
      if (ins.op == PO_ATOM_CMP || ins.op == PO_ATOM_REGEX) need_values[ins.col_a] = 1;
    }
    if (ins.col_b >= 0) { need_validity[ins.col_b] = 1; need_values[ins.col_b] = 1; }
  }
  int64_t b1000 = 0;
  for (int c = 0; c < ncols; ++c) {
    int32_t t = p->schema[c].type;
    if (need_values[c]) b1000 += value_bytes_x1000(t);
    if (need_validity[c] && p->schema[c].nullable) b1000 += 125;
  }
  p->bytes_per_row_x1000 = b1000;
  {
    auto bytes_of = [&](const std::vector<int>& vals, const std::vector<int>& valid) {
      int64_t b = 0;
      for (int c = 0; c < ncols; ++c) {
        int32_t t = p->schema[c].type;
        if (vals[c]) b += value_bytes_x1000(t);
        if (valid[c] && p->schema[c].nullable) b += 125;
      }
      return b;
    };
    std::vector<int> pv(ncols, 0), pn(ncols, 0), qv(ncols, 0), qn(ncols, 0);
    for (int i = 0; i < prog.n_instr; ++i) {
      const PredInstr& ins = prog.instr[i];
      if (ins.col_a >= 0) { pn[ins.col_a] = 1; if (ins.op == PO_ATOM_CMP || ins.op == PO_ATOM_REGEX) pv[ins.col_a] = 1; }
      if (ins.col_b >= 0) { pn[ins.col_b] = 1; pv[ins.col_b] = 1; }
    }
    for (const PairTask& pt : p->pair_tasks) { qv[pt.col_x] = qv[pt.col_y] = qn[pt.col_x] = qn[pt.col_y] = 1; }
    p->pred_bytes_x1000 = bytes_of(pv, pn);
    p->pair_bytes_x1000 = bytes_of(qv, qn);
  }
  p->launches_per_scan = (p->has_pred ? 1 : 0) + (int32_t)p->groups.size() + (p->pair_wgs.empty() ? 0 : 1) +
                         ((p->col_tasks.size() + p->pair_tasks.size()) ? 1 : 0);

  if (p->host_only) return DQ_OK;

  const size_t nct = p->col_tasks.size(), npt = p->pair_tasks.size();
  if (dq_status s = dmalloc(&p->d_col_tasks, nct * sizeof(ColTask))) return s;
  if (dq_status s = dmalloc(&p->d_pair_tasks, npt * sizeof(PairTask))) return s;
  if (dq_status s = dmalloc(&p->d_pair_wgs, p->pair_wgs.size() * sizeof(PairWG))) return s;
  if (!p->pair_wgs.empty())
    HIP_TRY(hipMemcpyAsync(p->d_pair_wgs, p->pair_wgs.data(), p->pair_wgs.size() * sizeof(PairWG),
                           hipMemcpyHostToDevice, p->stream));
  if (dq_status s = dmalloc(&p->d_pair_redo, p->pair_wgs.size() * kPairWaves * kMaxWG * sizeof(int32_t))) return s;
  if (dq_status s = dmalloc(&p->d_prog, sizeof(PredProgram))) return s;
  if (dq_status s = dmalloc(&p->d_col_part, nct * kMaxWG * sizeof(ColPartial))) return s;
  if (dq_status s = dmalloc(&p->d_pair_part, npt * kMaxWG * sizeof(CorrPartial))) return s;
  if (dq_status s = dmalloc(&p->d_pred_part, sizeof(PredPartial))) return s;
  if (dq_status s = dmalloc(&p->d_col_acc, nct * sizeof(ColPartial))) return s;
  if (dq_status s = dmalloc(&p->d_rare_dev, 2 * nct * sizeof(int64_t))) return s;
  if (nct) HIP_TRY(hipMemsetAsync(p->d_rare_dev, 0, 2 * nct * sizeof(int64_t), p->stream));
  p->str_long.assign(nct, 0);
  if (const char* e = std::getenv("DQ_STR_PATH")) p->str_path = std::strcmp(e, "fast") == 0 ? 1 : std::strcmp(e, "long") == 0 ? 2 : 0;
  if (nct && hipHostMalloc(reinterpret_cast<void**>(&p->h_rare), nct * sizeof(int64_t), hipHostMallocMapped) == hipSuccess) {
    std::memset(p->h_rare, 0, nct * sizeof(int64_t));
    void* dp = nullptr;
    if (hipHostGetDevicePointer(&dp, p->h_rare, 0) == hipSuccess) {
      p->d_rare = static_cast<int64_t*>(dp);
    } else {
      (void)hipHostFree(p->h_rare);
      p->h_rare = nullptr;
    }
  }
  (void)hipGetLastError();
  if (dq_status s = dmalloc(&p->d_hll_acc, (size_t)p->n_hll * kHllCopies * 512 * sizeof(uint32_t))) return s;
  if (dq_status s = dmalloc(&p->d_pair_acc, npt * sizeof(CorrPartial))) return s;
  if (dq_status s = dmalloc(&p->d_pred_acc, kPredAccCopies * sizeof(PredPartial))) return s;
  if (nct) HIP_TRY(hipMemcpyAsync(p->d_col_tasks, p->col_tasks.data(), nct * sizeof(ColTask), hipMemcpyHostToDevice, p->stream));
  if (npt) HIP_TRY(hipMemcpyAsync(p->d_pair_tasks, p->pair_tasks.data(), npt * sizeof(PairTask), hipMemcpyHostToDevice, p->stream));
  if (!p->regex_blob.empty()) {
    if (dq_status s = dmalloc(&p->d_regex, p->regex_blob.size() * sizeof(uint16_t))) return s;
    HIP_TRY(hipMemcpyAsync(p->d_regex, p->regex_blob.data(), p->regex_blob.size() * sizeof(uint16_t),
                           hipMemcpyHostToDevice, p->stream));
  }
  p->prog.regex = p->d_regex;
  p->prog.regex_words = (int32_t)p->regex_blob.size();
  HIP_TRY(hipMemcpyAsync(p->d_prog, &p->prog, sizeof(PredProgram), hipMemcpyHostToDevice, p->stream));
  if (dq_status s = reset_acc(p)) return s;
  HIP_TRY(hipStreamSynchronize(p->stream));
  return DQ_OK;
}



static void pred_columns(const dq_pred_node* pool, int32_t n_pred, int32_t idx, std::vector<int32_t>& cols,
                         int depth = 0) {
  if (idx < 0 || idx >= n_pred || depth > 64) return;
  const dq_pred_node& n = pool[idx];
  switch (n.kind) {
    case DQ_PRED_COLUMN: cols.push_back(n.a); return;
    case DQ_PRED_CMP: case DQ_PRED_AND: case DQ_PRED_OR: case DQ_PRED_COALESCE:
      pred_columns(pool, n_pred, n.a, cols, depth + 1);
      pred_columns(pool, n_pred, n.b, cols, depth + 1);
      return;
    case DQ_PRED_NOT: case DQ_PRED_IS_NULL: case DQ_PRED_IS_NOT_NULL: case DQ_PRED_REGEX:
      pred_columns(pool, n_pred, n.a, cols, depth + 1);
      return;
    default: return;
  }
}

static std::vector<int32_t> spec_columns(const dq_analyzer_spec& s, const dq_pred_node* pool, int32_t n_pred,
                                         int32_t ncols) {
  std::vector<int32_t> c;
  if (s.op == DQ_OP_CORRELATION) { c.push_back(s.col_a); c.push_back(s.col_b); }
  else if (s.op != DQ_OP_SIZE && s.op != DQ_OP_COMPLIANCE) c.push_back(s.col_a);
  pred_columns(pool, n_pred, s.pred_root, c);
  pred_columns(pool, n_pred, s.where_root, c);
  c.erase(std::remove_if(c.begin(), c.end(), [&](int32_t x) { return x < 0 || x >= ncols; }), c.end());
  std::sort(c.begin(), c.end());
  c.erase(std::unique(c.begin(), c.end()), c.end());
  return c;
}

struct PartInput {
  std::vector<dq_analyzer_spec> specs;
  std::vector<dq_column_desc> schema;
  std::vector<dq_pred_node> pool;
};

static void make_part_input(const std::vector<dq_analyzer_spec>& specs, const std::vector<dq_column_desc>& schema,
                            const dq_pred_node* pool, int32_t n_pred, const std::vector<int32_t>& spec_idx,
                            const std::vector<int32_t>& cols, PartInput& in) {
  const int32_t ncols = (int32_t)schema.size();
  std::vector<int32_t> local(ncols, -1);
  in.schema.clear();
  for (size_t j = 0; j < cols.size(); ++j) {
    local[cols[j]] = (int32_t)j;
    in.schema.push_back(schema[cols[j]]);
  }
  auto map = [&](int32_t c) { return c >= 0 && c < ncols ? local[c] : -1; };
  in.specs.clear();
  for (int32_t i : spec_idx) {
    dq_analyzer_spec sp = specs[i];
    if (sp.col_a >= 0) sp.col_a = map(sp.col_a);
    if (sp.col_b >= 0) sp.col_b = map(sp.col_b);
    in.specs.push_back(sp);
  }
  in.pool.assign(pool, pool + n_pred);
  for (dq_pred_node& n : in.pool)
    if (n.kind == DQ_PRED_COLUMN) n.a = map(n.a);
}

static dq_status plan_part_host(const dq_plan& parent, const dq_pred_node* pool, int32_t n_pred,
                                const std::vector<int32_t>& spec_idx, const std::vector<int32_t>& cols, bool probe,
                                dq_plan& q) {
  PartInput in;
  make_part_input(parent.specs, parent.schema, pool, n_pred, spec_idx, cols, in);
// ... 247 lines not shown

static dq_status check_view(const dq_column_desc& cd, const dq_column_view& v, int32_t c, int64_t n_rows) {
  const int32_t t = cd.type;
  if (v.reserved != 0) return set_error(DQ_E_INVALID, "dq_scan: column %d reserved field must be 0", c);
  if (n_rows > 0 && !v.values) return set_error(DQ_E_INVALID, "dq_scan: column %d has no values buffer", c);
  if (((uintptr_t)v.values & 15) != 0)
    return set_error(DQ_E_INVALID, "dq_scan: column %d values buffer must be 16-byte aligned", c);
  if (((uintptr_t)v.validity & 3) != 0)
    return set_error(DQ_E_INVALID, "dq_scan: column %d validity bitmap must be 4-byte aligned", c);
  if ((t == DQ_TYPE_UTF8 || t == DQ_TYPE_LARGE_UTF8) && n_rows > 0 && !v.offsets)
    return set_error(DQ_E_INVALID, "dq_scan: UTF8 column %d has no offsets", c);
  return DQ_OK;
}

extern "C" {

dq_status dq_scan(dq_plan* p, const dq_column_view* cols, int64_t n_rows, int64_t chunk_index) {
  if (!p) return set_error(DQ_E_INVALID, "dq_scan: plan is NULL");
  if (n_rows < 0) return set_error(DQ_E_INVALID, "dq_scan: n_rows < 0");
  if (n_rows >= (int64_t(1) << 31))
    return set_error(DQ_E_INVALID, "dq_scan: a chunk holds at most 2^31 - 1 rows (split larger inputs into chunks)");
  if (chunk_index != p->next_chunk)
    return set_error(DQ_E_INVALID, "dq_scan: chunk_index %lld out of order (expected %lld)", (long long)chunk_index,
                     (long long)p->next_chunk);
  const int32_t ncols = (int32_t)p->schema.size();
  if (ncols > 0 && !cols) return set_error(DQ_E_INVALID, "dq_scan: cols is NULL");
  HIP_TRY(hipSetDevice(p->device));
  if (!p->parts.empty()) {
    for (size_t k = 0; k < p->parts.size(); ++k) {
      for (int32_t c : p->part_cols[k])
        if (dq_status s = check_view(p->schema[c], cols[c], c, n_rows)) return s;
      if (p->parts[k]->next_chunk != chunk_index)
        return set_error(DQ_E_INVALID, "dq_scan: part %zu is at chunk %lld (expected %lld)", k,
                         (long long)p->parts[k]->next_chunk, (long long)chunk_index);
    }
    std::vector<dq_column_view> v;
    for (size_t k = 0; k < p->parts.size(); ++k) {
      v.resize(p->part_cols[k].size());
      for (size_t j = 0; j < v.size(); ++j) v[j] = cols[p->part_cols[k][j]];
      if (dq_status s = dq_scan(p->parts[k], v.data(), n_rows, chunk_index)) return s;
    }
    p->next_chunk++;
    p->total_rows += n_rows;
    return DQ_OK;
  }
  ScanCols sc{};
  for (int32_t c = 0; c < ncols; ++c)
    if (dq_status s = check_view(p->schema[c], cols[c], c, n_rows)) return s;
  for (int32_t c = 0; c < ncols; ++c) {
    const dq_column_view& v = cols[c];
    sc.values[c] = v.values;
    sc.validity[c] = p->schema[c].nullable ? reinterpret_cast<const uint32_t*>(v.validity) : nullptr;
    sc.offsets[c] = v.offsets;
  }
  p->next_chunk++;
  if (n_rows == 0) return DQ_OK;
  if (p->pred_jit_ref) {
    std::string note;
    if (hipFunction_t fn = pred_jit_poll(p->pred_jit_ref, 0, note)) {
      p->pred_jit = fn;
      p->pred_jit_note = note + " (compiled in the background; used from chunk " + std::to_string(chunk_index) + ")";
      p->pred_jit_ref.reset();
    } else if (!pred_jit_pending(p->pred_jit_ref)) {
      p->pred_jit_note = note;
      p->pred_jit_ref.reset();
    }
  }
  std::vector<dq_plan::Group> groups(p->groups);
  if (!p->pred_jit) groups.insert(groups.end(), p->pred_fused_groups.begin(), p->pred_fused_groups.end());

  const int64_t words = ceil_div(n_rows, 64);
  if (p->prog.n_bitmaps > 0 && words > p->where_cap_words) {
    HIP_TRY(hipStreamSynchronize(p->stream));
    for (int b = 0; b < p->prog.n_bitmaps; ++b) {
      if (p->d_where_bits[b]) (void)hipFree(p->d_where_bits[b]);
      p->d_where_bits[b] = nullptr;
      if (dq_status s = dmalloc(&p->d_where_bits[b], (size_t)words * 8 + 64)) return s;
    }
    p->where_cap_words = words;
  }
  ScanBitmaps bm{};
  for (int b = 0; b < kMaxWhere; ++b) bm.where_bits[b] = p->d_where_bits[b];
  bm.rare_rows = p->d_rare_dev;
  if ((!p->pair_wgs.empty() || p->pred_jit) && words + 1 > p->ones_cap_words) {
    HIP_TRY(hipStreamSynchronize(p->stream));
    if (p->d_ones) (void)hipFree(p->d_ones);
    p->d_ones = nullptr;
    if (dq_status s = dmalloc(&p->d_ones, (size_t)(words + 1) * 8)) return s;
    HIP_TRY(hipMemsetAsync(p->d_ones, 0xFF, (size_t)(words + 1) * 8, p->stream));
    p->ones_cap_words = words + 1;
  }

  int64_t min_launch = 0;
  for (const auto& g : groups) min_launch = min_launch ? std::min<int64_t>(min_launch, g.count) : g.count;
  if (!p->pair_wgs.empty()) {
    const int64_t wg = (int64_t)p->pair_wgs.size();
    min_launch = min_launch ? std::min<int64_t>(min_launch, wg) : wg;
  }
  const int64_t want = std::max<int64_t>(64, std::min<int64_t>(kMaxWG, kTargetWGs / std::max<int64_t>(1, min_launch)));
  auto size_ranges = [&](int64_t w, int64_t& rpr, int32_t& nr, int64_t min_rows) {
    w = std::min<int64_t>(w, std::max<int64_t>(1, n_rows / min_rows));
    nr = (int32_t)std::min<int64_t>(w, ceil_div(n_rows, kRowsPerIter));
    rpr = ceil_div(ceil_div(n_rows, nr), kRowsPerIter) * kRowsPerIter;
    nr = (int32_t)ceil_div(n_rows, rpr);
  };
  int32_t nr_col;
  int64_t rpr_col;
  size_ranges(want, rpr_col, nr_col, DQ_MIN_RANGE_ROWS);
  auto variant_scale = [](int32_t v) -> int32_t {
    return v == CV_UTF8_H || v == CV_LUTF8_H || v == CV_UTF8_HD || v == CV_LUTF8_HD ? 2 : 1;
  };
  auto variant_div = [](int32_t v) -> int32_t { return v == CV_F64_SH || v == CV_F64_H ? DQ_F64_HLL_DIV : 1; };
  auto variant_min_rows = [](int32_t v) -> int64_t {
    return v == CV_VALIDITY ? DQ_MIN_VALIDITY_RANGE_ROWS : DQ_MIN_RANGE_ROWS;
  };
  FinRanges fr{};
  std::vector<std::pair<int64_t, int32_t>> vr(groups.size());
  for (size_t gi = 0; gi < groups.size(); ++gi) {
    const auto& g = groups[gi];
    const int32_t sc_v = variant_scale(g.variant);
    const int64_t min_rows = variant_min_rows(g.variant);
    const int32_t div_v = variant_div(g.variant);
    if (sc_v == 1 && div_v == 1 && min_rows == DQ_MIN_RANGE_ROWS) {
      vr[gi] = {rpr_col, nr_col};
      continue;
    }
    size_ranges(std::max<int64_t>(64, std::min<int64_t>(kMaxWG, want * sc_v / div_v)), vr[gi].first, vr[gi].second, min_rows);
    if (vr[gi].second == nr_col && vr[gi].first == rpr_col) continue;
    if (fr.n >= kMaxFinRanges - 2) {
      vr[gi] = {rpr_col, nr_col};
      continue;
    }
    fr.first[fr.n] = g.first;
    fr.end[fr.n] = g.first + g.count;
    fr.nr[fr.n] = vr[gi].second;
    ++fr.n;
  }
  int32_t nr_pred = (int32_t)std::min<int64_t>(
      DQ_PRED_WGS, std::min<int64_t>(ceil_div(n_rows, kRowsPerIter), std::max<int64_t>(1, n_rows / DQ_MIN_RANGE_ROWS)));
  int64_t rpr_pred = ceil_div(ceil_div(n_rows, nr_pred), kRowsPerIter) * kRowsPerIter;
  nr_pred = (int32_t)ceil_div(n_rows, rpr_pred);

  const bool pair_ring = [&] {
    if (p->pair_wgs.empty() || !p->pair_all_f64) return false;
    for (const PairWG& wg : p->pair_wgs)
      for (const PairWaveTask& t : wg.wave)
        for (int c = 0; c < kPairPos; ++c)
          if (((uintptr_t)sc.values[t.cols[c]] & 15u) != 0) return false;
    return true;
  }();
  int64_t rpr_pair = rpr_col;
  int32_t nr_pair = nr_col;
  if (!p->pair_wgs.empty() && DQ_PAIR_ONE_ROUND) {
    int32_t& res = p->pair_resident[pair_ring ? 1 : 0];
    if (res == 0) {
      int32_t per_cu = 0, cus = 0;
      HIP_TRY(pair_scan_residency(p->pair_all_f64, pair_ring, p->pair_minmax, &per_cu));
      HIP_TRY(hipDeviceGetAttribute(&cus, hipDeviceAttributeMultiprocessorCount, p->device));
      res = std::max<int32_t>(1, per_cu * cus);
    }
    const int64_t per_round = std::max<int64_t>(1, res / (int64_t)p->pair_wgs.size());
    size_ranges(std::min<int64_t>(kMaxWG, per_round), rpr_pair, nr_pair, DQ_MIN_RANGE_ROWS);
    if (nr_pair != nr_col && p->pair_fused_count > 0) {
      fr.first[fr.n] = p->pair_fused_first;
      fr.end[fr.n] = p->pair_fused_first + p->pair_fused_count;
      fr.nr[fr.n] = nr_pair;
      ++fr.n;
    }
  }
  if (p->pred_jit && p->pred_fused_count > 0) {
    fr.first[fr.n] = p->pred_fused_first;
    fr.end[fr.n] = p->pred_fused_first + p->pred_fused_count;
    fr.nr[fr.n] = nr_pred;
    ++fr.n;
  }

  if (p->has_pred) {
    if (dq_status s = timed(p, 0, p->stream, [&] {
          if (p->pred_jit) {
            PredJitArgs a{};
            for (size_t i = 0; i < p->pred_jit_cols.size(); ++i) {
              a.values[i] = reinterpret_cast<const char*>(sc.values[p->pred_jit_cols[i]]);
              const uint32_t* vb = sc.validity[p->pred_jit_cols[i]];
              a.validity[i] = vb ? vb : reinterpret_cast<const uint32_t*>(p->d_ones);
            }
            for (int b = 0; b < kMaxWhere && b < 8; ++b) a.where_bits[b] = bm.where_bits[b];
            a.n_rows = n_rows;
            a.rows_per_range = rpr_pred;
            a.acc_t = reinterpret_cast<unsigned long long*>(p->d_pred_acc->t);
            a.acc_nn = reinterpret_cast<unsigned long long*>(p->d_pred_acc->nn);
            a.col_part = reinterpret_cast<char*>(p->d_col_part);
            a.hll_acc = p->d_hll_acc;
            for (size_t h = 0; h < p->pred_jit_hll_task.size(); ++h) {
              a.hll_task[h] = p->pred_jit_hll_task[h];
              a.hll_slot[h] = p->pred_jit_hll_slot[h];
            }
            return pred_jit_launch(p->pred_jit, a, nr_pred, p->stream);
          }
          const int32_t lds = kWaves * 128 * (p->prog.stack_depth + p->prog.n_roots + p->prog.n_counters) +
                              ((p->prog.regex_words * 2 + 15) & ~15);
          return launch_pred_scan(p->d_prog, sc, bm, n_rows, rpr_pred, nr_pred, p->d_pred_acc, lds, p->stream,
                                  p->prog.regex_words > 0);
        }))
      return s;
  }
  auto str_long_of = [&](const dq_plan::Group& g) -> bool {
    if (g.variant != CV_UTF8_H && g.variant != CV_LUTF8_H && g.variant != CV_UTF8_HD && g.variant != CV_LUTF8_HD)
      return false;
    if (p->str_path != 0) return p->str_path == 2;
    const int64_t rows = p->total_rows > 0 ? p->total_rows : p->prev_rows;
    bool any = false;
    for (int32_t t = g.first; t < g.first + g.count; ++t) {
      if (p->h_rare && rows > 0) p->str_long[t] = __atomic_load_n(p->h_rare + t, __ATOMIC_RELAXED) * 4096 > rows;
      any = any || p->str_long[t];
    }
    return any;
  };
  for (size_t gi = 0; gi < groups.size(); ++gi) {
    const auto& g = groups[gi];
    if (dq_status s = timed(p, 16 + g.variant, p->stream, [&] {
          return launch_column_scan(g.variant, p->d_col_tasks + g.first, g.count, g.first, sc, bm, n_rows,
                                    vr[gi].first, vr[gi].second, p->d_col_part, p->d_hll_acc, str_long_of(g),
                                    p->stream);
        }))
      return s;
  }
  if (!p->pair_wgs.empty()) {
    const bool ring = pair_ring;
    if (dq_status s = timed(p, 2, p->stream, [&] {
          return launch_pair_scan(p->d_pair_wgs, (int32_t)p->pair_wgs.size(), sc, bm, p->d_ones, n_rows, rpr_pair,
                                  nr_pair, p->d_pair_part, p->d_col_part, p->d_pair_redo, p->pair_all_f64, ring,
                                  p->pair_minmax, p->stream);
        }))
      return s;
  }
  if (dq_status s = timed(p, 3, p->stream, [&] {
        return launch_finalize((int32_t)p->col_tasks.size(), nr_col, p->d_col_part, p->d_col_acc,
                               (int32_t)p->pair_tasks.size(), nr_pair, p->d_pair_part, p->d_pair_acc,
                               0 , nr_pred, p->d_pred_part, p->d_pred_acc,
                               fr, p->d_rare_dev, p->d_rare, p->stream);
      }))
    return s;
  p->total_rows += n_rows;
  return DQ_OK;
}

dq_status dq_finish(dq_plan* p, dq_state* out) {
  if (!p) return set_error(DQ_E_INVALID, "dq_finish: plan is NULL");
  if (!out && !p->specs.empty()) return set_error(DQ_E_INVALID, "dq_finish: out is NULL");
  HIP_TRY(hipSetDevice(p->device));
  if (!p->parts.empty()) {
    std::vector<dq_state> tmp;
    for (size_t k = 0; k < p->parts.size(); ++k) {
      tmp.assign(p->part_specs[k].size(), dq_state{});
      if (dq_status s = dq_finish(p->parts[k], tmp.data())) return s;
      for (size_t j = 0; j < tmp.size(); ++j) out[p->part_specs[k][j]] = tmp[j];
    }
    return DQ_OK;
  }
  std::vector<ColPartial> col(p->col_tasks.size());
  std::vector<uint32_t> hll((size_t)p->n_hll * kHllCopies * 512);
  std::vector<CorrPartial> pair(p->pair_tasks.size());
  PredPartial pred{};
  std::vector<PredPartial> pred_copies(p->has_pred ? kPredAccCopies : 0);
  const size_t b_col = col.size() * sizeof(ColPartial), b_hll = hll.size() * sizeof(uint32_t),
               b_pair = pair.size() * sizeof(CorrPartial), b_pred = pred_copies.size() * sizeof(PredPartial);
  const size_t o_hll = b_col, o_pair = o_hll + b_hll, o_pred = o_pair + b_pair, b_all = o_pred + b_pred;
  if (b_all > p->h_stage_bytes) {
    if (p->h_stage) (void)hipHostFree(p->h_stage);
    p->h_stage = nullptr;
    p->h_stage_bytes = 0;
    if (hipHostMalloc(reinterpret_cast<void**>(&p->h_stage), b_all, hipHostMallocDefault) == hipSuccess) {
      p->h_stage_bytes = b_all;
    } else {
      (void)hipGetLastError();
      p->h_stage = nullptr;
    }
  }
  char* const hs = p->h_stage;
  void* const dst_col = hs ? (void*)hs : (void*)col.data();
  void* const dst_hll = hs ? (void*)(hs + o_hll) : (void*)hll.data();
  void* const dst_pair = hs ? (void*)(hs + o_pair) : (void*)pair.data();
  void* const dst_pred = hs ? (void*)(hs + o_pred) : (void*)pred_copies.data();
  if (b_col) HIP_TRY(hipMemcpyAsync(dst_col, p->d_col_acc, b_col, hipMemcpyDeviceToHost, p->stream));
  if (b_hll) HIP_TRY(hipMemcpyAsync(dst_hll, p->d_hll_acc, b_hll, hipMemcpyDeviceToHost, p->stream));
  if (b_pair) HIP_TRY(hipMemcpyAsync(dst_pair, p->d_pair_acc, b_pair, hipMemcpyDeviceToHost, p->stream));
  if (b_pred) HIP_TRY(hipMemcpyAsync(dst_pred, p->d_pred_acc, b_pred, hipMemcpyDeviceToHost, p->stream));
  HIP_TRY(hipStreamSynchronize(p->stream));
  if (hs) {
    if (b_col) std::memcpy(col.data(), hs, b_col);
    if (b_hll) std::memcpy(hll.data(), hs + o_hll, b_hll);
    if (b_pair) std::memcpy(pair.data(), hs + o_pair, b_pair);
    if (b_pred) std::memcpy(pred_copies.data(), hs + o_pred, b_pred);
  }
  for (const PredPartial& c : pred_copies)
    for (int k = 0; k < kMaxCounters; ++k) {
      pred.t[k] += c.t[k];
      pred.nn[k] += c.nn[k];
    }
  if (dq_status s = resolve_timing(p)) return s;

  const int64_t rows = p->total_rows;
  const double nan = std::numeric_limits<double>::quiet_NaN();
  const double inf = std::numeric_limits<double>::infinity();
  auto f64_sum = [&](const ColPartial& c) {
    double v = c.sum;
    if (c.pinf_count > 0) v += inf;
    if (c.ninf_count > 0) v += -inf;
    return v;
  };
  for (size_t i = 0; i < p->specs.size(); ++i) {
    const SpecOut& o = p->outs[i];
    dq_state& s = out[i];
    std::memset(&s, 0, sizeof(s));
    s.op = o.op;
    auto set1 = [&](bool v) { s.has_value[0] = s.has_value[1] = v ? 1 : 0; };
    const ColPartial* c = o.col_task >= 0 ? &col[o.col_task] : nullptr;
    switch (o.op) {
      case DQ_OP_SIZE:
        if (o.ctr_b >= 0) { s.u.size.num_matches = pred.t[o.ctr_b]; set1(pred.nn[o.ctr_b] > 0); }
        else { s.u.size.num_matches = rows; set1(true); }
        break;
      case DQ_OP_COMPLETENESS:
        if (o.has_where) {
          s.u.ratio.num_matches = pred.t[o.ctr_a];
          s.u.ratio.count = pred.t[o.ctr_b];
          s.has_value[0] = rows > 0;
          s.has_value[1] = pred.nn[o.ctr_b] > 0;
        } else {
          s.u.ratio.num_matches = c ? c->count : rows;
          s.u.ratio.count = rows;
          s.has_value[0] = rows > 0;
          s.has_value[1] = 1;
        }
        break;
      case DQ_OP_COMPLIANCE:
      case DQ_OP_PATTERN_MATCH:
        s.u.ratio.num_matches = pred.t[o.ctr_a];
        s.has_value[0] = pred.nn[o.ctr_a] > 0;
        if (o.has_where) { s.u.ratio.count = pred.t[o.ctr_b]; s.has_value[1] = pred.nn[o.ctr_b] > 0; }
        else { s.u.ratio.count = rows; s.has_value[1] = 1; }
        break;
      case DQ_OP_SUM:
        if (is_decimal(o.col_type)) {
          s.integral = 2;
          s.u.sum.dec_scale = DQ_DECIMAL_SCALE(o.col_type);
          s.u.sum.dec_digits = std::min(38, DQ_DECIMAL_PRECISION(o.col_type) + 10);
          s.u.sum.partial = c->isum;
          s.u.sum.partial_hi = c->isum_hi;
          s.u.sum.guard = c->sum;
          if (!dec_sum_value(c->isum, c->isum_hi, c->sum, s.u.sum.dec_scale, s.u.sum.dec_digits, s.u.sum.sum))
            s.u.sum.sum = nan;
        } else {
          s.u.sum.sum = is_floating(o.col_type) ? f64_sum(*c) : (double)c->isum;
          s.integral = !is_floating(o.col_type);
          s.u.sum.partial = s.integral ? c->isum : 0;
        }
        set1(c->count > 0);
        break;
      case DQ_OP_MEAN:
        if (is_decimal(o.col_type)) {
          s.integral = 2;
          s.u.mean.dec_scale = DQ_DECIMAL_SCALE(o.col_type);
          s.u.mean.dec_digits = std::min(38, DQ_DECIMAL_PRECISION(o.col_type) + 10);
          s.u.mean.partial = c->isum;
          s.u.mean.partial_hi = c->isum_hi;
// ... 78 lines not shown
  if (!p->parts.empty()) {
    for (dq_plan* q : p->parts)
      if (dq_status s = dq_plan_reset(q)) return s;
    p->total_rows = 0;
    p->next_chunk = 0;
    return DQ_OK;
  }
  return reset_acc(p);
}

void dq_plan_destroy(dq_plan* p) {
  if (!p) return;
  (void)hipSetDevice(p->device);
  for (dq_plan* q : p->parts) dq_plan_destroy(q);
  p->parts.clear();
  if (p->stream) (void)hipStreamSynchronize(p->stream);
  free_plan_mem(p);
  if (p->own_stream && p->stream) (void)hipStreamDestroy(p->stream);
  delete p;
}

int64_t dq_plan_bytes_per_row_x1000(const dq_plan* p) { return p ? p->bytes_per_row_x1000 : 0; }

dq_status dq_plan_enable_timing(dq_plan* p, int32_t on) {
  if (!p) return set_error(DQ_E_INVALID, "dq_plan_enable_timing: plan is NULL");
  HIP_TRY(hipSetDevice(p->device));
  for (dq_plan* q : p->parts)
    if (dq_status s = dq_plan_enable_timing(q, on)) return s;
  if (dq_status s = resolve_timing(p)) return s;
  p->timing = on != 0;
  for (int k = 0; k < dq_plan::kTimers; ++k) { p->kernel_ms[k] = 0; p->kernel_launches[k] = 0; }
  return DQ_OK;
}

dq_status dq_plan_kernel_time(dq_plan* p, int32_t kernel, double* total_ms, int64_t* launches) {
  if (!p || kernel < 0 || kernel >= dq_plan::kTimers || !total_ms || !launches)
    return set_error(DQ_E_INVALID, "dq_plan_kernel_time: bad argument");
  HIP_TRY(hipSetDevice(p->device));
  if (!p->parts.empty()) {
    double ms = 0.0;
    int64_t n = 0;
    for (dq_plan* q : p->parts) {
      double m = 0.0;
      int64_t k = 0;
      if (dq_status s = dq_plan_kernel_time(q, kernel, &m, &k)) return s;
      ms += m;
      n += k;
    }
    *total_ms = ms;
    *launches = n;
    return DQ_OK;
  }
  if (dq_status s = resolve_timing(p)) return s;
  if (kernel == 1) {
    double ms = 0;
    int64_t n = 0;
    for (int k = 16; k < dq_plan::kTimers; ++k) { ms += p->kernel_ms[k]; n += p->kernel_launches[k]; }
    *total_ms = ms;
    *launches = n;
  } else {
    *total_ms = p->kernel_ms[kernel];
    *launches = p->kernel_launches[kernel];
  }
  return DQ_OK;
}

int64_t dq_plan_variant_bytes_per_row_x1000(const dq_plan* p, int32_t variant) {
  if (!p) return 0;
  int64_t b = 0;
  for (const dq_plan* q : p->parts) b += dq_plan_variant_bytes_per_row_x1000(q, variant);
  const size_t n_run = p->col_tasks.size() - (size_t)p->n_fused;
  for (size_t i = 0; i < n_run; ++i) {
    const ColTask& t = p->col_tasks[i];
    if (t.variant != variant) continue;
    const dq_column_desc& cd = p->schema[t.col];
    if (t.variant != CV_VALIDITY) b += value_bytes_x1000(cd.type);
    if (cd.nullable) b += 125;
    if (t.where >= 0) b += 125;
  }
  return b;
}
int32_t dq_plan_num_launches(const dq_plan* p) { return p ? p->launches_per_scan : 0; }

dq_status dq_plan_create_time(const dq_plan* p, double* total_ms, double* pred_jit_ms) {
  if (!p) return set_error(DQ_E_INVALID, "dq_plan_create_time: plan is NULL");
  if (total_ms) *total_ms = p->create_ms;
  if (pred_jit_ms) *pred_jit_ms = p->pred_jit_ms;
  return DQ_OK;
}

int64_t dq_plan_explain(const dq_analyzer_spec* specs, int32_t n_specs, const dq_column_desc* schema, int32_t n_cols,
                        const dq_pred_node* pred_pool, int32_t n_pred, const char* const* patterns, int32_t n_patterns,
                        const dq_plan_options* opts, char* out, int64_t cap) {
  if (n_specs < 0 || (n_specs > 0 && !specs)) return set_error(DQ_E_INVALID, "dq_plan_explain: bad specs");
  if (n_cols < 0 || n_cols > kMaxSchemaCols || (n_cols > 0 && !schema))
    return set_error(DQ_E_INVALID, "dq_plan_explain: bad schema (at most %d columns)", kMaxSchemaCols);
  if (n_pred < 0 || (n_pred > 0 && !pred_pool)) return set_error(DQ_E_INVALID, "dq_plan_explain: bad predicate pool");
  if (n_patterns < 0 || (n_patterns > 0 && !patterns)) return set_error(DQ_E_INVALID, "dq_plan_explain: bad patterns");
  for (int32_t k = 0; k < n_patterns; ++k)
    if (!patterns[k]) return set_error(DQ_E_INVALID, "dq_plan_explain: pattern %d is NULL", k);
  for (int32_t c = 0; c < n_cols; ++c)
    if (!type_valid(schema[c].type))
      return set_error(DQ_E_TYPE, "dq_plan_explain: column %d has unknown type %d", c, schema[c].type);
  if (cap < 0 || (cap > 0 && !out)) return set_error(DQ_E_INVALID, "dq_plan_explain: bad output buffer");
  std::unique_ptr<dq_plan> holder(new dq_plan());
  dq_plan& plan = *holder;
  plan.host_only = true;
  plan.schema.assign(schema, schema + n_cols);
  plan.specs.assign(specs, specs + n_specs);
  for (int32_t k = 0; k < n_patterns; ++k) plan.patterns.emplace_back(patterns[k]);
  if (opts) {
    if (opts->struct_size < (int32_t)(2 * sizeof(int32_t))) return set_error(DQ_E_INVALID, "dq_plan_explain: bad options");
    if (opts->pred_pass < DQ_PRED_PASS_AUTO || opts->pred_pass > DQ_PRED_PASS_COMPILED)
      return set_error(DQ_E_INVALID, "dq_plan_explain: unknown pred_pass %d", opts->pred_pass);
    plan.pred_pass = opts->pred_pass;
  }
  std::string t;
  char line[256];
  g_capacity = false;
  dq_status st = n_cols <= kMaxCols ? build_plan(&plan, pred_pool, n_pred)
                                    : cap_error("more than %d columns in one plan", kMaxCols);
  if (st == DQ_OK) {
    std::snprintf(line, sizeof line, "plan: %d analyzers, %d columns, %d launches per scan\n", n_specs, n_cols,
                  plan.launches_per_scan);
    t += line;
    t += explain_text(plan);
  } else {
    if (!g_capacity) return st;
    std::string why = g_err;
    std::vector<std::vector<int32_t>> ps, pc;
    if (dq_status s2 = partition_specs(plan, pred_pool, n_pred, ps, pc)) return s2;
    std::snprintf(line, sizeof line, "plan: %d analyzers, %d columns, over one plan's capacity (%s): %zu fused plans\n",
                  n_specs, n_cols, why.c_str(), ps.size());
    t += line;
    for (size_t k = 0; k < ps.size(); ++k) {
      std::unique_ptr<dq_plan> q(new dq_plan());
      if (dq_status s2 = plan_part_host(plan, pred_pool, n_pred, ps[k], pc[k], false, *q)) return s2;
      std::snprintf(line, sizeof line, "--- part %zu: %zu analyzers, %zu columns, %d launches per scan\n", k,
                    ps[k].size(), pc[k].size(), q->launches_per_scan);
      t += line;
      t += "analyzers:";
      for (int32_t i : ps[k]) t += " " + std::to_string(i);
      t += "\ncolumns:";
      for (int32_t c : pc[k]) t += " " + std::to_string(c);
      t += "\n" + explain_text(*q);
    }
  }
  if (cap > 0) {
    const size_t n = std::min((size_t)cap - 1, t.size());
    std::memcpy(out, t.data(), n);
    out[n] = '\0';
  }
  return (int64_t)t.size() + 1;
}

int32_t dq_plan_pred_wait(dq_plan* p, int32_t timeout_ms) {
  if (!p) return set_error(DQ_E_INVALID, "dq_plan_pred_wait: plan is NULL");
  if (!p->parts.empty()) {
    int32_t all = 1, any_pred = 0;
    for (dq_plan* q : p->parts) {
      if (!q->has_pred) continue;
      any_pred = 1;
      const int32_t r = dq_plan_pred_wait(q, timeout_ms);
      if (r < 0) return r;
      all &= r;
    }
// ... 48 lines not shown
```

### deequ_amd/runner.py

```python
from __future__ import annotations

import ctypes
import json
import math
from typing import Dict, Iterable, List, Optional, Sequence

from . import _lib as L
from .analyzers import Analyzer, PlanBuilder, Preconditions, data_schema
from .metrics import DoubleMetric, UnsupportedOnGpuPathException
from .predicates import UnsupportedPredicate
from .states import State
from .table import Table


def _chunks(data) -> List[Table]:
    return [data] if isinstance(data, Table) else list(data)


class ScanPlan:

    def __init__(self, analyzers: Sequence[Analyzer], schema, device: Optional[int] = None, pred_pass: str = "auto"):
        import torch

        self.analyzers = list(analyzers)
        b = PlanBuilder(schema)
        specs = (L.AnalyzerSpec * max(1, len(self.analyzers)))()
        for i, a in enumerate(self.analyzers):
            op, ca, cb, pr, wr = a._lower(b)
            specs[i].op, specs[i].col_a, specs[i].col_b, specs[i].pred_root, specs[i].where_root = op, ca, cb, pr, wr
        self.columns = list(b.columns)
        sch = b.schema_ctypes()
        pool, npred = b.pool.as_ctypes()
        if device is None:
            device = torch.cuda.current_device()
        self.device = device
        self._specs, self._sch, self._pool = specs, sch, pool
        handle = ctypes.c_void_p()
        pats, npats = b.pool.patterns_ctypes()
        self._pats = pats
        opts = L.PlanOptions(ctypes.sizeof(L.PlanOptions), L.PRED_PASS[pred_pass])
        L.check(L.lib.dq_plan_create_opts(specs, len(self.analyzers), sch, len(self.columns), pool, npred, pats, npats,
                                          ctypes.byref(opts), device, ctypes.byref(handle)))
        self.handle = handle
        self.chunk = 0
        with torch.cuda.device(device):
            L.check(L.lib.dq_plan_set_stream(self.handle, ctypes.c_void_p(torch.cuda.current_stream().cuda_stream)))

    def bytes_per_row(self) -> float:
        return L.lib.dq_plan_bytes_per_row_x1000(self.handle) / 1000.0

    def num_launches(self) -> int:
        return L.lib.dq_plan_num_launches(self.handle)

    def enable_timing(self, on: bool = True) -> None:
        L.check(L.lib.dq_plan_enable_timing(self.handle, 1 if on else 0))

    def variant_bytes_per_row(self, variant: int) -> float:
        return L.lib.dq_plan_variant_bytes_per_row_x1000(self.handle, variant) / 1000.0

    def pred_compiled(self):
        buf = ctypes.create_string_buffer(2048)
        on = L.lib.dq_plan_pred_compiled(self.handle, buf, len(buf))
        return bool(on), buf.value.decode("utf-8", "replace")

    def pred_wait(self, timeout_ms: int = -1) -> bool:
        r = L.lib.dq_plan_pred_wait(self.handle, timeout_ms)
        if r < 0:
            L.check(r)
        return bool(r)

    def create_time(self):
        total, jit = ctypes.c_double(), ctypes.c_double()
        L.check(L.lib.dq_plan_create_time(self.handle, ctypes.byref(total), ctypes.byref(jit)))
        return total.value, jit.value

    def kernel_bytes_per_row(self, kernel: int) -> float:
        return L.lib.dq_plan_kernel_bytes_per_row_x1000(self.handle, kernel) / 1000.0

    def kernel_time(self, kernel: int):
        ms, n = ctypes.c_double(), ctypes.c_int64()
        L.check(L.lib.dq_plan_kernel_time(self.handle, kernel, ctypes.byref(ms), ctypes.byref(n)))
        return ms.value, n.value

    def scan(self, table: Table) -> None:
        views = (L.ColumnView * max(1, len(self.columns)))()
        for i, name in enumerate(self.columns):
            views[i] = table.columns[name].view()
        L.check(L.lib.dq_scan(self.handle, views, table.num_rows, self.chunk))
        self.chunk += 1

    def finish(self) -> List[L.State]:
        out = (L.State * max(1, len(self.analyzers)))()
        L.check(L.lib.dq_finish(self.handle, out))
        return [out[i] for i in range(len(self.analyzers))]

    def reset(self) -> None:
        L.check(L.lib.dq_plan_reset(self.handle))
        self.chunk = 0

    def close(self) -> None:
        if self.handle:
            L.lib.dq_plan_destroy(self.handle)
            self.handle = None

    def __del__(self):
        try:
            self.close()
        except Exception:
            pass


def _lower_all(analyzers: Sequence[Analyzer], schema):
    b = PlanBuilder(schema)
    specs = (L.AnalyzerSpec * max(1, len(analyzers)))()
    for i, a in enumerate(analyzers):
        op, ca, cb, pr, wr = a._lower(b)
        specs[i].op, specs[i].col_a, specs[i].col_b, specs[i].pred_root, specs[i].where_root = op, ca, cb, pr, wr
    return b, specs


def _explain(b: PlanBuilder, specs, n_specs: int, pred_pass: str):
    sch = b.schema_ctypes()
    pool, npred = b.pool.as_ctypes()
    pats, npats = b.pool.patterns_ctypes()
    opts = L.PlanOptions(ctypes.sizeof(L.PlanOptions), L.PRED_PASS[pred_pass])
    args = (specs, n_specs, sch, len(b.columns), pool, npred, pats, npats, ctypes.byref(opts))
    n = L.lib.dq_plan_explain(*args, None, 0)
    if n < 0:
        return int(n), L.lib.dq_last_error().decode("utf-8", "replace")
    buf = ctypes.create_string_buffer(int(n))
    L.lib.dq_plan_explain(*args, buf, n)
    return L.DQ_OK, buf.value.decode("utf-8", "replace")


def explain(analyzers: Sequence[Analyzer], schema, pred_pass: str = "auto") -> str:
    b, specs = _lower_all(analyzers, schema)
    rc, text = _explain(b, specs, len(analyzers), pred_pass)
    L.check(rc)
    return text


def scan_results(data, analyzers: Sequence[Analyzer], pred_pass: str = "auto") -> List[L.State]:
    chunks = _chunks(data)
    plan = ScanPlan(analyzers, chunks[0].schema, pred_pass=pred_pass)
    try:
        for t in chunks:
            plan.scan(t)
        return plan.finish()
    finally:
        plan.close()


def scan_states(data, analyzers: Sequence[Analyzer], pred_pass: str = "auto") -> Dict[Analyzer, Optional[State]]:
    res = scan_results(data, analyzers, pred_pass)
    return {a: a._from_result(r) for a, r in zip(analyzers, res)}


def gpu_eligible(analyzer: Analyzer, schema) -> Optional[Exception]:
    try:
        b, specs = _lower_all([analyzer], schema)
    except UnsupportedPredicate as e:
        return e
    except Exception:
        return None
    rc, msg = _explain(b, specs, 1, "auto")
    if rc == L.DQ_E_UNSUPPORTED:
        return UnsupportedPredicate(msg)
    return None
# ... 173 lines not shown
```

### include/dqscan.h

```cpp
#ifndef DQSCAN_H
#define DQSCAN_H

#include <stdint.h>

#ifdef __cplusplus
extern "C" {
#endif

#define DQ_ABI_VERSION 6

typedef int32_t dq_status;
#define DQ_OK 0
#define DQ_E_INVALID (-1)
#define DQ_E_TYPE (-2)
#define DQ_E_UNSUPPORTED (-3)
#define DQ_E_HIP (-4)
#define DQ_E_OOM (-5)
#define DQ_E_STATE (-6)

enum dq_type {
  DQ_TYPE_F64 = 1,
  DQ_TYPE_I64 = 2,
  DQ_TYPE_I32 = 3,
  DQ_TYPE_UTF8 = 4,
// ... 105 lines not shown
};
#endif

typedef struct dq_host_column {
  int32_t type;
  int32_t nullable;
  int64_t n_rows;
  const void* values;
  const uint8_t* validity;
  const void* offsets;
  int64_t value_bytes, validity_bytes, offset_bytes;
  int64_t offset_base;
  int32_t validity_bit;
  int32_t reserved;
} dq_host_column;
dq_status dq_arrow_import(const struct ArrowSchema* schema, const struct ArrowArray* array, dq_host_column* out);
typedef struct dq_uploader dq_uploader;
dq_status dq_uploader_create(int32_t device, int32_t n_slots, int64_t slot_bytes, int32_t host_threads,
                             dq_uploader** out);
dq_status dq_upload(dq_uploader* u, const dq_host_column* cols, int32_t n_cols, dq_column_view* dev_views);
dq_status dq_upload_fence(dq_uploader* u, void* hip_stream);
dq_status dq_upload_release(dq_uploader* u, void* hip_stream);
dq_status dq_upload_sync(dq_uploader* u);
void dq_uploader_destroy(dq_uploader* u);

typedef struct dq_state {
  int32_t op;
  uint8_t has_value[2];
  uint8_t integral;
  uint8_t reserved;
  union {
    struct { int64_t num_matches; } size;
    struct { int64_t num_matches; int64_t count; } ratio;
    struct { double sum; int64_t partial; int64_t partial_hi; double guard; int32_t dec_scale, dec_digits; } sum;
    struct { double sum; int64_t count; int64_t partial; int64_t partial_hi; double guard; int32_t dec_scale, dec_digits; } mean;
    struct { double n, avg, m2; } stddev;
    struct { double value; } minmax;
    struct { double n, x_avg, y_avg, ck, x_mk, y_mk; } corr;
    struct { int64_t words[52]; } hll;
    struct { int64_t num_null, num_fractional, num_integral, num_boolean, num_string; } dtype;
  } u;
} dq_state;

typedef struct dq_plan dq_plan;

int32_t dq_abi_version(void);
const char* dq_last_error(void);

dq_status dq_plan_create(const dq_analyzer_spec* specs, int32_t n_specs, const dq_column_desc* schema,
                         int32_t n_cols, const dq_pred_node* pred_pool, int32_t n_pred, int32_t device,
                         dq_plan** out);
dq_status dq_plan_create_ex(const dq_analyzer_spec* specs, int32_t n_specs, const dq_column_desc* schema,
                            int32_t n_cols, const dq_pred_node* pred_pool, int32_t n_pred,
                            const char* const* patterns, int32_t n_patterns, int32_t device, dq_plan** out);
enum dq_pred_pass { DQ_PRED_PASS_AUTO = 0, DQ_PRED_PASS_INTERPRETER = 1, DQ_PRED_PASS_COMPILED = 2 };
typedef struct dq_plan_options {
  int32_t struct_size;
  int32_t pred_pass;
  int32_t reserved[6];
} dq_plan_options;
dq_status dq_plan_create_opts(const dq_analyzer_spec* specs, int32_t n_specs, const dq_column_desc* schema,
                              int32_t n_cols, const dq_pred_node* pred_pool, int32_t n_pred,
                              const char* const* patterns, int32_t n_patterns, const dq_plan_options* opts,
                              int32_t device, dq_plan** out);
dq_status dq_regex_info(const char* pattern, int32_t mode, int32_t* n_states, int32_t* n_classes);
dq_status dq_regex_match_host(const char* pattern, int32_t mode, const uint8_t* data, const int64_t* offsets,
                              int64_t n, uint8_t* out);
typedef struct dq_pred_pool dq_pred_pool;
dq_status dq_pred_pool_create(const char* const* names, const int32_t* types, int32_t n_cols, dq_pred_pool** out);
dq_status dq_pred_pool_add(dq_pred_pool* pool, const char* sql, int32_t* root);
dq_status dq_pred_pool_add_regex(dq_pred_pool* pool, int32_t column, const char* pattern, int32_t mode, int32_t* root);
int32_t dq_pred_pool_size(const dq_pred_pool* pool);
const dq_pred_node* dq_pred_pool_nodes(const dq_pred_pool* pool);
int32_t dq_pred_pool_num_patterns(const dq_pred_pool* pool);
const char* const* dq_pred_pool_patterns(const dq_pred_pool* pool);
void dq_pred_pool_destroy(dq_pred_pool* pool);
dq_status dq_plan_set_stream(dq_plan* plan, void* hip_stream);
dq_status dq_scan(dq_plan* plan, const dq_column_view* cols, int64_t n_rows, int64_t chunk_index);
dq_status dq_finish(dq_plan* plan, dq_state* out_states);
dq_status dq_plan_reset(dq_plan* plan);
void dq_plan_destroy(dq_plan* plan);
int64_t dq_plan_bytes_per_row_x1000(const dq_plan* plan);
int32_t dq_plan_num_launches(const dq_plan* plan);
dq_status dq_plan_enable_timing(dq_plan* plan, int32_t on);
dq_status dq_plan_kernel_time(dq_plan* plan, int32_t kernel, double* total_ms, int64_t* launches);
int64_t dq_plan_variant_bytes_per_row_x1000(const dq_plan* plan, int32_t variant);
int64_t dq_plan_kernel_bytes_per_row_x1000(const dq_plan* plan, int32_t kernel);
int32_t dq_plan_pred_compiled(const dq_plan* plan, char* note, int32_t cap);
int32_t dq_plan_pred_wait(dq_plan* plan, int32_t timeout_ms);
int64_t dq_plan_explain(const dq_analyzer_spec* specs, int32_t n_specs, const dq_column_desc* schema, int32_t n_cols,
                        const dq_pred_node* pred_pool, int32_t n_pred, const char* const* patterns, int32_t n_patterns,
                        const dq_plan_options* opts, char* out, int64_t cap);
dq_status dq_plan_create_time(const dq_plan* plan, double* total_ms, double* pred_jit_ms);

typedef struct dq_freq_table dq_freq_table;
typedef struct dq_freq_summary {
  int64_t num_groups;
  int64_t num_unique;
  int64_t num_values;
  double entropy;
} dq_freq_summary;
dq_status dq_freq_build(const int32_t* types, int32_t n_cols, const dq_column_view* cols, const int64_t* chunk_rows,
                        int32_t n_chunks, int32_t device, void* hip_stream, dq_freq_table** out);
dq_status dq_freq_merge(const dq_freq_table* a, const dq_freq_table* b, dq_freq_table** out);
dq_status dq_freq_summarize(const dq_freq_table* t, int64_t num_rows, dq_freq_summary* out);
int64_t dq_freq_num_groups(const dq_freq_table* t);
dq_status dq_freq_export(const dq_freq_table* t, uint64_t* keys, int64_t* counts, int64_t cap);
void dq_freq_destroy(dq_freq_table* t);
#define DQ_MAX_QUANTILES 8
dq_status dq_approx_quantiles(int32_t type, const dq_column_view* cols, const int64_t* chunk_rows, int32_t n_chunks,
                              const double* quantiles, int32_t n_q, double relative_error, int32_t device,
                              void* hip_stream, double* out, int64_t* count);
dq_status dq_quantile_digest(int32_t type, const dq_column_view* cols, const int64_t* chunk_rows, int32_t n_chunks,
                             double relative_error, int32_t device, void* hip_stream, double* values, int64_t* ranks,
                             int64_t cap, int64_t* n_samples, int64_t* count);
dq_status dq_freq_top(const dq_freq_table* t, int32_t n, uint64_t* keys, int64_t* counts, uint64_t* rep_rows,
                      int32_t* n_out);
dq_status dq_mutual_information(const int32_t* types, const dq_column_view* cols, const int64_t* chunk_rows,
                                int32_t n_chunks, int64_t num_rows, int32_t device, void* hip_stream, double* value,
                                int32_t* defined);

dq_status dq_state_merge(const dq_state* a, const dq_state* b, dq_state* out);
dq_status dq_state_combine(const dq_state* a, const dq_state* b, dq_state* out);
dq_status dq_state_merge_n(const dq_state* a, const dq_state* b, int32_t n, dq_state* out);
dq_status dq_state_combine_n(const dq_state* a, const dq_state* b, int32_t n, dq_state* out);
int32_t dq_state_is_defined(const dq_state* s);
dq_status dq_state_metric(const dq_state* s, double* out);
dq_status dq_hll_estimate(const int64_t* words52, double* out);

int64_t dq_state_to_bytes(const dq_state* s, uint8_t* buf, int64_t cap);
dq_status dq_state_from_bytes(int32_t op, const uint8_t* buf, int64_t len, dq_state* out);
int32_t dq_state_identifier(const char* analyzer_to_string_utf8);

#ifdef __cplusplus
}
#endif

#endif
```

Before: 30.40 billion rows/s.

## Track integer HLL distinct values in a dense bitmap window instead of hashing

Integer columns that feed HLL get a 64K-value window. Values inside the window set a bit in a shared/global bitmap instead of being hashed into HLL registers, and the bitmap is folded into the HLL state at finish. For i64/i32 the window base is picked automatically by sampling the min and max in the first chunk, while i8/i16 use a static window. Only out-of-window values are reloaded and hashed. This is meant to cut the per-row xxhash and register-update cost for the 4 int64 columns. In exchange it adds ballots, atomics on LDS bitmap words, extra shared memory per workgroup, and a finish kernel.

```diff
diff --git a/deequ_amd/_lib.py b/deequ_amd/_lib.py
--- a/deequ_amd/_lib.py
+++ b/deequ_amd/_lib.py
@@ -93,6 +93,12 @@
 class ColumnView(ctypes.Structure):
     _fields_ = [("values", ctypes.c_void_p), ("validity", ctypes.c_void_p), ("offsets", ctypes.c_void_p),
                 ("reserved", ctypes.c_int64)]
+
+
+class IntWindow(ctypes.Structure):
+    _fields_ = [("column", ctypes.c_int32), ("has_where", ctypes.c_int32), ("on", ctypes.c_int32),
+                ("off_for_run", ctypes.c_int32), ("is_static", ctypes.c_int32), ("reserved", ctypes.c_int32),
+                ("base", ctypes.c_int64), ("rows_in", ctypes.c_int64), ("rows_out", ctypes.c_int64)]
 
 
 class _Size(ctypes.Structure):
@@ -244,6 +250,11 @@
     L.dq_plan_bytes_per_row_x1000.argtypes = [c.c_void_p]
     L.dq_plan_num_launches.restype = c.c_int32
     L.dq_plan_num_launches.argtypes = [c.c_void_p]
+    if hasattr(L, "dq_plan_int_window"):
+        L.dq_plan_int_window_count.restype = c.c_int32
+        L.dq_plan_int_window_count.argtypes = [c.c_void_p]
+        L.dq_plan_int_window.restype = c.c_int32
+        L.dq_plan_int_window.argtypes = [c.c_void_p, c.c_int32, P(IntWindow)]
     L.dq_plan_enable_timing.restype = c.c_int32
     L.dq_plan_enable_timing.argtypes = [c.c_void_p, c.c_int32]
     L.dq_plan_kernel_time.restype = c.c_int32
@@ -292,6 +303,7 @@
     "dq_plan_set_stream", "dq_freq_build", "dq_freq_merge", "dq_freq_summarize", "dq_freq_num_groups",
     "dq_freq_export", "dq_freq_destroy", "dq_mutual_information", "dq_approx_quantiles", "dq_quantile_digest", "dq_freq_top", "dq_scan", "dq_finish",
     "dq_plan_reset", "dq_plan_destroy", "dq_plan_bytes_per_row_x1000", "dq_plan_num_launches",
+    "dq_plan_int_window_count", "dq_plan_int_window",
     "dq_plan_enable_timing", "dq_plan_kernel_time", "dq_plan_variant_bytes_per_row_x1000",
     "dq_plan_kernel_bytes_per_row_x1000", "dq_plan_pred_compiled", "dq_plan_pred_wait",
     "dq_state_merge", "dq_state_combine", "dq_state_merge_n", "dq_state_combine_n", "dq_state_is_defined", "dq_state_metric", "dq_hll_estimate",
diff --git a/deequ_amd/csrc/dq_device.h b/deequ_amd/csrc/dq_device.h
--- a/deequ_amd/csrc/dq_device.h
+++ b/deequ_amd/csrc/dq_device.h
@@ -60,8 +60,27 @@
   int32_t where;
   int32_t hll_slot;
   int32_t arg;
-  int32_t pad[3];
-};
+  int32_t win;
+  int32_t pad[2];
+};
+
+constexpr int kWinBits = 16;
+constexpr int64_t kWinValues = int64_t(1) << kWinBits;
+constexpr int kWinWords = (int)(kWinValues / 32);
+constexpr int64_t kWinMargin = 4096;
+constexpr int64_t kWinOffShare = 64;
+enum IntWinMode : int32_t { WIN_AUTO = 1, WIN_STATIC = 2 };
+struct IntWin {
+  int64_t base;
+  int64_t vmin, vmax;
+  unsigned long long rows_in, rows_out;
+  unsigned long long prev_in, prev_out;
+  int32_t mode;
+  int32_t on;
+  int32_t off_for_run;
+  int32_t pad;
+};
+static_assert(sizeof(IntWin) == 72, "IntWin layout");
 
 struct PairTask {
   int32_t col_x, col_y;
@@ -181,6 +200,11 @@
   const void* offsets[kMaxCols];
 };
 
+struct ScanWindows {
+  IntWin* win;
+  uint32_t* bits;
+};
+
 struct ScanBitmaps {
   uint64_t* where_bits[kMaxWhere];
   int64_t* rare_rows;
diff --git a/deequ_amd/csrc/dq_kernels.hip b/deequ_amd/csrc/dq_kernels.hip
--- a/deequ_amd/csrc/dq_kernels.hip
+++ b/deequ_amd/csrc/dq_kernels.hip
@@ -368,6 +368,95 @@
   }
 }
 
+template <int K> struct KindT { using T = double; };
+template <> struct KindT<CK_I64> { using T = int64_t; };
+template <> struct KindT<CK_I32> { using T = int32_t; };
+template <> struct KindT<CK_F32> { using T = float; };
+template <> struct KindT<CK_I16> { using T = int16_t; };
+template <> struct KindT<CK_I8> { using T = int8_t; };
+
+template <int KIND, bool STATS>
+__device__ __forceinline__ void numeric_block_win(const double (&x)[8], const uint64_t (&bits)[8], const uint64_t (&m)[8],
+                                                  double shift, ColStats& s, LaneMoments& a, int32_t* regs,
+                                                  uint32_t* wbits, uint64_t wbase, __amdgpu_buffer_rsrc_t vr, int32_t vo,
+                                                  int64_t& out_w) {
+  using T = typename KindT<KIND>::T;
+  uint64_t any_out = 0;
+#pragma unroll
+  for (int j = 0; j < 8; ++j) {
+    if (STATS) masked_moments<true, false>(a, s.fmin, s.fmax, x[j], bits[j], shift, m[j], m[j]);
+    const uint64_t d = bits[j] - wbase;
+    const bool in = d < (uint64_t)kWinValues;
+    any_out |= __builtin_amdgcn_ballot_w64(!in) & m[j];
+    if (lane_bit(m[j]) && in) atomicOr(&wbits[(uint32_t)d >> 5], 1u << ((uint32_t)d & 31u));
+  }
+  if (any_out != 0) {
+#pragma unroll 1
+    for (int j = 0; j < 8; ++j) {
+      uint64_t b;
+      if constexpr (sizeof(T) == 8) {
+        const auto w2 = __builtin_amdgcn_raw_buffer_load_b64(vr, vo + j * 512, 0, 0);
+        b = ((uint64_t)w2[1] << 32) | w2[0];
+      } else if constexpr (sizeof(T) == 4) {
+        b = (uint64_t)(int64_t)(int32_t)__builtin_amdgcn_raw_buffer_load_b32(vr, vo + j * 256, 0, 0);
+      } else if constexpr (sizeof(T) == 2) {
+        b = (uint64_t)(int64_t)(int16_t)__builtin_amdgcn_raw_buffer_load_b16(vr, vo + j * 128, 0, 0);
+      } else {
+        b = (uint64_t)(int64_t)(int8_t)__builtin_amdgcn_raw_buffer_load_b8(vr, vo + j * 64, 0, 0);
+      }
+      uint64_t mj = m[0];
+#pragma unroll
+      for (int k = 1; k < 8; ++k) mj = j == k ? m[k] : mj;
+      const uint64_t om = __builtin_amdgcn_ballot_w64(b - wbase >= (uint64_t)kWinValues) & mj;
+      out_w += __builtin_popcountll(om);
+      if (lane_bit(om)) hll_update(regs, ck_bytes(KIND) <= 4 ? xxh64_int((uint32_t)b) : xxh64_long(b));
+    }
+  }
+}
+
+template <int KIND>
+__device__ __forceinline__ void window_sample(__amdgpu_buffer_rsrc_t vr, const uint32_t* validity, const uint32_t* mask,
+                                              int64_t base, int32_t rem, int32_t vo, IntWin* win) {
+  using T = typename KindT<KIND>::T;
+  int64_t lo = INT64_MAX, hi = INT64_MIN;
+#pragma unroll 1
+  for (int j = 0; j < 8; ++j) {
+    const int32_t left = rem - 64 * j;
+    if (left <= 0) break;
+    const int64_t r = base + 64 * j;
+    uint64_t mj = ~0ull;
+    {
+      const int64_t w = r >> 5;
+      const bool two = left > 32;
+      if (validity) mj = ((uint64_t)(two ? ((const_u32s)validity)[w + 1] : 0u) << 32) | ((const_u32s)validity)[w];
+      if (mask) mj &= ((uint64_t)(two ? ((const_u32s)mask)[w + 1] : 0u) << 32) | ((const_u32s)mask)[w];
+      if (left < 64) mj &= (1ull << left) - 1ull;
+    }
+    if (mj == 0) continue;
+    int64_t b;
+    if constexpr (sizeof(T) == 8) {
+      const auto w2 = __builtin_amdgcn_raw_buffer_load_b64(vr, vo + j * 512, 0, 0);
+      b = (int64_t)(((uint64_t)w2[1] << 32) | w2[0]);
+    } else {
+      b = (int64_t)(int32_t)__builtin_amdgcn_raw_buffer_load_b32(vr, vo + j * 256, 0, 0);
+    }
+    if (lane_bit(mj)) {
+      lo = b < lo ? b : lo;
+      hi = b > hi ? b : hi;
+    }
+  }
+#pragma unroll
+  for (int k = 32; k >= 1; k >>= 1) {
+    const int64_t ol = __shfl_xor(lo, k), oh = __shfl_xor(hi, k);
+    lo = ol < lo ? ol : lo;
+    hi = oh > hi ? oh : hi;
+  }
+  if ((threadIdx.x & 63) == 0 && lo <= hi) {
+    atomicMin(reinterpret_cast<long long*>(&win->vmin), (long long)lo);
+    atomicMax(reinterpret_cast<long long*>(&win->vmax), (long long)hi);
+  }
+}
+
 template <int KIND, bool STATS, bool HLL>
 __device__ __forceinline__ void float_block_checked(__amdgpu_buffer_rsrc_t vr, const uint32_t* validity,
                                                     const uint32_t* mask, int64_t base, int32_t rem, int32_t vo,
@@ -424,18 +513,13 @@
   }
 }
 
-template <int K> struct KindT { using T = double; };
-template <> struct KindT<CK_I64> { using T = int64_t; };
-template <> struct KindT<CK_I32> { using T = int32_t; };
-template <> struct KindT<CK_F32> { using T = float; };
-template <> struct KindT<CK_I16> { using T = int16_t; };
-template <> struct KindT<CK_I8> { using T = int8_t; };
-
 template <int KIND, bool STATS, bool HLL>
 __device__ void numeric_range(const void* values, const uint32_t* validity, const uint32_t* mask,
-                              int64_t row0, int64_t row1, ColStats& s, int32_t* regs) {
+                              int64_t row0, int64_t row1, ColStats& s, int32_t* regs, IntWin* win = nullptr,
+                              uint32_t* wbits = nullptr, bool win_on = false, int64_t win_base = 0) {
   using T = typename KindT<KIND>::T;
   constexpr bool kLazy = ck_float(KIND) && STATS;
+  constexpr bool kWin = HLL && !ck_float(KIND);
   const int lane = threadIdx.x & 63;
   const int wave = __builtin_amdgcn_readfirstlane(threadIdx.x >> 6);
   const T* v = reinterpret_cast<const T*>(values);
@@ -447,47 +531,30 @@
   const double shift = STATS ? range_shift_of<KIND>(vr, validity, mask, row0, row1, lane) : 0.0;
   int32_t qmin = 0;
   const int32_t nr = (int32_t)(row1 - row0);
-  for (int32_t rb = 0; rb < nr; rb += kRowsPerIter) {
-    const int64_t base = row0 + rb + wave * 512;
-    const int32_t rem = nr - rb - wave * 512;
-    const bool full = rb + kRowsPerIter <= nr;
-    uint64_t bits[8], m[8];
-    double x[8];
-    const int32_t vo = (rb + wave * 512 + lane) * (int32_t)sizeof(T);
-#pragma unroll
-    for (int j = 0; j < 8; ++j) {
-      if constexpr (sizeof(T) == 8) {
-        const auto w2 = __builtin_amdgcn_raw_buffer_load_b64(vr, vo + j * 512, 0, 2 );
-        bits[j] = ((uint64_t)w2[1] << 32) | w2[0];
-        if (KIND == CK_F64) x[j] = __builtin_bit_cast(double, bits[j]);
-        else x[j] = __builtin_fma((double)(int32_t)w2[1], 4294967296.0, (double)w2[0]);
-      } else if constexpr (KIND == CK_F32) {
-        const uint32_t w = __builtin_amdgcn_raw_buffer_load_b32(vr, vo + j * 256, 0, 2 );
-        bits[j] = w;
-        x[j] = (double)__builtin_bit_cast(float, w);
-      } else {
-        int32_t w;
-        if constexpr (sizeof(T) == 4) w = (int32_t)__builtin_amdgcn_raw_buffer_load_b32(vr, vo + j * 256, 0, 2 );
-        else if constexpr (sizeof(T) == 2) w = (int16_t)__builtin_amdgcn_raw_buffer_load_b16(vr, vo + j * 128, 0, 2 );
-        else w = (int8_t)__builtin_amdgcn_raw_buffer_load_b8(vr, vo + j * 64, 0, 2 );
-        bits[j] = (uint64_t)(int64_t)w;
-        x[j] = (double)w;
-      }
-    }
-    block_masks(validity, mask, base, rem, full, m);
-    uint64_t nf_any = 0;
-    if constexpr (ck_float(KIND) && !kLazy) {
-#pragma unroll
-      for (int j = 0; j < 8; ++j) nf_any |= __builtin_amdgcn_ballot_w64(!__builtin_isfinite(x[j])) & m[j];
-    }
-    if (ck_float(KIND) && !kLazy && nf_any != 0) {
-      float_block_checked<KIND, STATS, HLL>(vr, validity, mask, base, rem, vo, shift, s, a, regs, cnt_w, nan_v, pinf_v,
-                                            ninf_v);
+  int64_t out_w = 0;
+  if constexpr (kWin && sizeof(T) >= 4) {
+    if ( win && !win_on && win->mode == WIN_AUTO && !win->off_for_run)
+      window_sample<KIND>(vr, validity, mask, row0 + wave * 512, nr - wave * 512,
+                          (wave * 512 + lane) * (int32_t)sizeof(T), win);
+  }
+  if constexpr (kWin) {
+    if (win_on) {
+#define DQ_NUMERIC_LOOP_WIN true
+#include "dq_numeric_loop.inc"
+#undef DQ_NUMERIC_LOOP_WIN
+      if (lane == 0 && cnt_w > 0) {
+        atomicAdd(&win->rows_in, (unsigned long long)(cnt_w - out_w));
+        if (out_w) atomicAdd(&win->rows_out, (unsigned long long)out_w);
+      }
     } else {
-#pragma unroll
-      for (int j = 0; j < 8; ++j) cnt_w += __builtin_popcountll(m[j]);
-      numeric_block<KIND, STATS, HLL>(x, bits, m, shift, s, a, regs, qmin);
-    }
+#define DQ_NUMERIC_LOOP_WIN false
+#include "dq_numeric_loop.inc"
+#undef DQ_NUMERIC_LOOP_WIN
+    }
+  } else {
+#define DQ_NUMERIC_LOOP_WIN false
+#include "dq_numeric_loop.inc"
+#undef DQ_NUMERIC_LOOP_WIN
   }
   if constexpr (kLazy) {
     __shared__ int32_t redo;
@@ -1130,7 +1197,8 @@
 template <int V, bool LONG>
 __device__ __forceinline__ void run_variant(const ColTask& t, const ScanCols& cols, const uint32_t* mask, int64_t row0,
                                             int64_t row1, int64_t n_rows, ColStats& s, int32_t* regs,
-                                            const uint64_t* p5, uint32_t* dq, uint32_t* rare, uint32_t* cls) {
+                                            const uint64_t* p5, uint32_t* dq, uint32_t* rare, uint32_t* cls,
+                                            IntWin* win, uint32_t* wbits, bool win_on, int64_t win_base) {
   const void* v = cols.values[t.col];
   const uint32_t* val = cols.validity[t.col];
   if constexpr (V == CV_VALIDITY) validity_range(val, mask, row0, row1, s);
@@ -1138,20 +1206,20 @@
   else if constexpr (V == CV_F64_SH) numeric_range<CK_F64, true, true>(v, val, mask, row0, row1, s, regs);
   else if constexpr (V == CV_F64_H) numeric_range<CK_F64, false, true>(v, val, mask, row0, row1, s, regs);
   else if constexpr (V == CV_I64_S) numeric_range<CK_I64, true, false>(v, val, mask, row0, row1, s, regs);
-  else if constexpr (V == CV_I64_SH) numeric_range<CK_I64, true, true>(v, val, mask, row0, row1, s, regs);
-  else if constexpr (V == CV_I64_H) numeric_range<CK_I64, false, true>(v, val, mask, row0, row1, s, regs);
+  else if constexpr (V == CV_I64_SH) numeric_range<CK_I64, true, true>(v, val, mask, row0, row1, s, regs, win, wbits, win_on, win_base);
+  else if constexpr (V == CV_I64_H) numeric_range<CK_I64, false, true>(v, val, mask, row0, row1, s, regs, win, wbits, win_on, win_base);
   else if constexpr (V == CV_I32_S) numeric_range<CK_I32, true, false>(v, val, mask, row0, row1, s, regs);
-  else if constexpr (V == CV_I32_SH) numeric_range<CK_I32, true, true>(v, val, mask, row0, row1, s, regs);
-  else if constexpr (V == CV_I32_H) numeric_range<CK_I32, false, true>(v, val, mask, row0, row1, s, regs);
+  else if constexpr (V == CV_I32_SH) numeric_range<CK_I32, true, true>(v, val, mask, row0, row1, s, regs, win, wbits, win_on, win_base);
+  else if constexpr (V == CV_I32_H) numeric_range<CK_I32, false, true>(v, val, mask, row0, row1, s, regs, win, wbits, win_on, win_base);
   else if constexpr (V == CV_F32_S) numeric_range<CK_F32, true, false>(v, val, mask, row0, row1, s, regs);
   else if constexpr (V == CV_F32_SH) numeric_range<CK_F32, true, true>(v, val, mask, row0, row1, s, regs);
   else if constexpr (V == CV_F32_H) numeric_range<CK_F32, false, true>(v, val, mask, row0, row1, s, regs);
   else if constexpr (V == CV_I16_S) numeric_range<CK_I16, true, false>(v, val, mask, row0, row1, s, regs);
-  else if constexpr (V == CV_I16_SH) numeric_range<CK_I16, true, true>(v, val, mask, row0, row1, s, regs);
-  else if constexpr (V == CV_I16_H) numeric_range<CK_I16, false, true>(v, val, mask, row0, row1, s, regs);
+  else if constexpr (V == CV_I16_SH) numeric_range<CK_I16, true, true>(v, val, mask, row0, row1, s, regs, win, wbits, win_on, win_base);
+  else if constexpr (V == CV_I16_H) numeric_range<CK_I16, false, true>(v, val, mask, row0, row1, s, regs, win, wbits, win_on, win_base);
   else if constexpr (V == CV_I8_S) numeric_range<CK_I8, true, false>(v, val, mask, row0, row1, s, regs);
-  else if constexpr (V == CV_I8_SH) numeric_range<CK_I8, true, true>(v, val, mask, row0, row1, s, regs);
-  else if constexpr (V == CV_I8_H) numeric_range<CK_I8, false, true>(v, val, mask, row0, row1, s, regs);
+  else if constexpr (V == CV_I8_SH) numeric_range<CK_I8, true, true>(v, val, mask, row0, row1, s, regs, win, wbits, win_on, win_base);
+  else if constexpr (V == CV_I8_H) numeric_range<CK_I8, false, true>(v, val, mask, row0, row1, s, regs, win, wbits, win_on, win_base);
   else if constexpr (V == CV_F64_D) float_dtype_range(reinterpret_cast<const double*>(v), val, mask, row0, row1, s);
   else if constexpr (V == CV_F32_D) float_dtype_range(reinterpret_cast<const float*>(v), val, mask, row0, row1, s);
   else if constexpr (V == CV_BOOL) bool_range(reinterpret_cast<const uint32_t*>(v), val, mask, row0, row1, s, regs);
@@ -1187,7 +1255,7 @@
                                                          int32_t part_base, ScanCols cols, ScanBitmaps bm,
                                                          int64_t n_rows, int64_t rows_per_range,
                                                          ColPartial* __restrict__ partials,
-                                                         uint32_t* __restrict__ hll_acc) {
+                                                         uint32_t* __restrict__ hll_acc, ScanWindows sw) {
   constexpr bool kHll = !(V == CV_VALIDITY || V == CV_F64_S || V == CV_I64_S || V == CV_I32_S || V == CV_F64_D ||
                          V == CV_UTF8_D || V == CV_LUTF8_D || V == CV_F32_S || V == CV_I16_S || V == CV_I8_S ||
                          V == CV_F32_D || V == CV_BOOL || V == CV_D128_S || V == CV_D128_D);
@@ -1201,9 +1269,25 @@
   constexpr bool kCls = DQ_STR_CLS && (V == CV_UTF8_H || V == CV_LUTF8_H) && !LONG;
   __shared__ __attribute__((aligned(16))) uint32_t clsbuf[kCls ? kWaves * kClsWords : 4];
   __shared__ ColStats red[kWaves];
+  constexpr bool kIntHll = V == CV_I64_SH || V == CV_I64_H || V == CV_I32_SH || V == CV_I32_H || V == CV_I16_SH ||
+                           V == CV_I16_H || V == CV_I8_SH || V == CV_I8_H;
+  __shared__ uint32_t wbits[kIntHll ? kWinWords : 1];
   const int32_t ti = blockIdx.x % ntasks;
   const int32_t range = blockIdx.x / ntasks;
   const ColTask t = tasks[ti];
+  IntWin* win = nullptr;
+  bool win_on = false;
+  int64_t win_base = 0;
+  if constexpr (kIntHll) {
+    if (sw.win && t.win >= 0) {
+      win = sw.win + t.win;
+      win_on = win->on != 0;
+      win_base = win->base;
+    }
+    if (win_on) {
+      for (int i = threadIdx.x; i < kWinWords; i += kBlock) wbits[i] = 0;
+    }
+  }
   const int64_t row0 = (int64_t)range * rows_per_range;
   int64_t row1 = row0 + rows_per_range;
   if (row1 > n_rows) row1 = n_rows;
@@ -1224,7 +1308,7 @@
   const uint32_t* mask = t.where >= 0 ? reinterpret_cast<const uint32_t*>(bm.where_bits[t.where]) : nullptr;
   const int32_t wv = kStr ? __builtin_amdgcn_readfirstlane(threadIdx.x >> 6) : 0;
   run_variant<V, LONG>(t, cols, mask, row0, row1, n_rows, s, regs, p5, dfq + wv * kDefFields * kDCap, rare + wv,
-                       clsbuf + (kCls ? wv * kClsWords : 0));
+                       clsbuf + (kCls ? wv * kClsWords : 0), win, wbits, win_on, win_base);
   block_reduce_store(s, partials + (size_t)(part_base + ti) * kMaxWG + range, red);
   if constexpr (kStr) {
     if (threadIdx.x == 0 && bm.rare_rows) {
@@ -1249,6 +1333,39 @@
     for (int i = threadIdx.x; i < 512; i += kBlock) {
       const uint32_t v = (uint32_t)(regs[i] + 1);
       if (v > __builtin_nontemporal_load(dst + i)) atomicMax(dst + i, v);
+    }
+    if constexpr (kIntHll) {
+      if (win_on) {
+        uint32_t* gb = sw.bits + (size_t)t.win * kWinWords;
+        for (int i = threadIdx.x; i < kWinWords; i += kBlock) {
+          const uint32_t w = wbits[i];
+          if (w != 0 && (w & ~__builtin_nontemporal_load(gb + i)) != 0) atomicOr(gb + i, w);
+        }
+      }
+    }
+  }
+}
+
+__global__ __launch_bounds__(kBlock) void dq_window_finish(const ColTask* __restrict__ tasks, int32_t ntasks,
+                                                           const IntWin* __restrict__ win,
+                                                           const uint32_t* __restrict__ win_bits,
+                                                           uint32_t* __restrict__ hll_acc) {
+  const int32_t ti = blockIdx.x;
+  if (ti >= ntasks) return;
+  const ColTask t = tasks[ti];
+  if (t.win < 0 || t.hll_slot < 0) return;
+  const bool is64 = t.variant == CV_I64_SH || t.variant == CV_I64_H;
+  const uint64_t base = (uint64_t)win[t.win].base;
+  const uint32_t* gb = win_bits + (size_t)t.win * kWinWords;
+  uint32_t* dst = hll_acc + (size_t)t.hll_slot * kHllCopies * 512;
+  for (int i = threadIdx.x; i < kWinWords; i += kBlock) {
+    uint32_t w = gb[i];
+    while (w != 0) {
+      const int b = __builtin_ctz(w);
+      w &= w - 1;
+      const uint64_t v = base + (uint64_t)(i * 32 + b);
+      const uint64_t x = is64 ? xxh64_long(v) : xxh64_int((uint32_t)v);
+      atomicMax(dst + (uint32_t)(x >> 55), (uint32_t)(hll_q_exact(x) + 1));
     }
   }
 }
@@ -1760,7 +1877,8 @@
                                                       CorrPartial* __restrict__ pair_acc, int32_t has_pred,
                                                       int32_t nranges_pred, const PredPartial* __restrict__ pred_part,
                                                       PredPartial* __restrict__ pred_acc, FinRanges fr,
-                                                      int64_t* __restrict__ rare_dev, int64_t* rare_host) {
+                                                      int64_t* __restrict__ rare_dev, int64_t* rare_host,
+                                                      const ColTask* __restrict__ tasks, IntWin* win) {
   __shared__ ColStats cs[kBlock];
   __shared__ CorrStats ps[kBlock];
   const int b = blockIdx.x, tid = threadIdx.x;
@@ -1785,6 +1903,25 @@
         rare_dev[ncol + b] = rare_dev[b];
         __hip_atomic_store(rare_host + b, rare_dev[b], __ATOMIC_RELAXED, __HIP_MEMORY_SCOPE_SYSTEM);
       }
+      if (win && tasks[b].win >= 0) {
+        IntWin& w = win[tasks[b].win];
+        if (w.mode == WIN_AUTO) {
+          if (w.on) {
+            const unsigned long long din = w.rows_in - w.prev_in, dout = w.rows_out - w.prev_out;
+            if (dout * (unsigned long long)kWinOffShare > din + dout) { w.on = 0; w.off_for_run = 1; }
+          } else if (!w.off_for_run && w.vmin <= w.vmax) {
+            const uint64_t span = (uint64_t)w.vmax - (uint64_t)w.vmin;
+            if (span <= (uint64_t)(kWinValues - 1 - 2 * kWinMargin)) {
+              w.base = (int64_t)((uint64_t)w.vmin - ((uint64_t)(kWinValues - 1) - span) / 2);
+              w.on = 1;
+            } else {
+              w.off_for_run = 1;
+            }
+          }
+          w.prev_in = w.rows_in;
+          w.prev_out = w.rows_out;
+        }
+      }
     }
   } else if (b < ncol + npair) {
     const int p = b - ncol;
@@ -1825,8 +1962,16 @@
   }
 }
 
-__global__ void dq_init_acc(ColPartial* col_acc, int32_t ncol, CorrPartial* pair_acc, int32_t npair, int64_t* rare_dev) {
+__global__ void dq_init_acc(ColPartial* col_acc, int32_t ncol, CorrPartial* pair_acc, int32_t npair, int64_t* rare_dev,
+                            IntWin* win, int32_t nwin) {
   const int i = blockIdx.x * blockDim.x + threadIdx.x;
+  if (i < nwin) {
+    IntWin& w = win[i];
+    w.vmin = INT64_MAX;
+    w.vmax = INT64_MIN;
+    w.rows_in = w.rows_out = w.prev_in = w.prev_out = 0;
+    w.off_for_run = 0;
+  }
   if (i < ncol) {
     ColStats s;
     stats_init(s);
@@ -1854,25 +1999,25 @@
 template <int V>
 static void launch_v(const ColTask* tasks, int32_t ntasks, int32_t part_base, const ScanCols& cols,
                      const ScanBitmaps& bm, int64_t n_rows, int64_t rows_per_range, int32_t nranges,
-                     ColPartial* partials, uint32_t* hll_acc, bool long_str, hipStream_t st) {
+                     ColPartial* partials, uint32_t* hll_acc, const ScanWindows& sw, bool long_str, hipStream_t st) {
   constexpr bool kStrHll = V == CV_UTF8_H || V == CV_LUTF8_H || V == CV_UTF8_HD || V == CV_LUTF8_HD;
   if constexpr (kStrHll) {
     if (long_str) {
       hipLaunchKernelGGL((dq_column_scan<V, true>), dim3((uint32_t)ntasks * (uint32_t)nranges), dim3(kBlock), 0, st,
-                         tasks, ntasks, part_base, cols, bm, n_rows, rows_per_range, partials, hll_acc);
+                         tasks, ntasks, part_base, cols, bm, n_rows, rows_per_range, partials, hll_acc, sw);
       return;
     }
   }
   hipLaunchKernelGGL(dq_column_scan<V>, dim3((uint32_t)ntasks * (uint32_t)nranges), dim3(kBlock), 0, st, tasks, ntasks,
-                     part_base, cols, bm, n_rows, rows_per_range, partials, hll_acc);
+                     part_base, cols, bm, n_rows, rows_per_range, partials, hll_acc, sw);
 }
 
 hipError_t launch_column_scan(int32_t variant, const ColTask* tasks, int32_t ntasks, int32_t part_base,
                               const ScanCols& cols, const ScanBitmaps& bm, int64_t n_rows, int64_t rows_per_range,
-                              int32_t nranges, ColPartial* partials, uint32_t* hll_acc, bool long_str, hipStream_t st) {
+                              int32_t nranges, ColPartial* partials, uint32_t* hll_acc, const ScanWindows& sw, bool long_str, hipStream_t st) {
 #define DQ_V(V)                                                                                            \
   case V:                                                                                                  \
-    launch_v<V>(tasks, ntasks, part_base, cols, bm, n_rows, rows_per_range, nranges, partials, hll_acc, long_str, \
+    launch_v<V>(tasks, ntasks, part_base, cols, bm, n_rows, rows_per_range, nranges, partials, hll_acc, sw, long_str, \
                 st);                                                                                       \
     break;
   switch (variant) {
@@ -1892,21 +2037,30 @@
 hipError_t launch_finalize(int32_t ncol, int32_t nranges_col, const ColPartial* col_part, ColPartial* col_acc,
                            int32_t npair, int32_t nranges_pair, const CorrPartial* pair_part, CorrPartial* pair_acc,
                            int32_t has_pred, int32_t nranges_pred, const PredPartial* pred_part, PredPartial* pred_acc,
-                           const FinRanges& fr, int64_t* rare_dev, int64_t* rare_host, hipStream_t st) {
+                           const FinRanges& fr, int64_t* rare_dev, int64_t* rare_host, const ColTask* tasks, IntWin* win,
+                           hipStream_t st) {
   const uint32_t nb = (uint32_t)(ncol + npair + (has_pred ? 1 : 0));
   if (nb == 0) return hipSuccess;
   hipLaunchKernelGGL(dq_finalize, dim3(nb), dim3(kBlock), 0, st, ncol, nranges_col, col_part, col_acc, npair,
                      nranges_pair, pair_part, pair_acc, has_pred, nranges_pred, pred_part, pred_acc, fr, rare_dev,
-                     rare_host);
+                     rare_host, tasks, win);
   return hipGetLastError();
 }
 
 hipError_t launch_init_acc(ColPartial* col_acc, int32_t ncol, CorrPartial* pair_acc, int32_t npair, int64_t* rare_dev,
-                           hipStream_t st) {
+                           IntWin* win, int32_t nwin, hipStream_t st) {
   const int n = ncol > npair ? ncol : npair;
   if (n == 0) return hipSuccess;
-  hipLaunchKernelGGL(dq_init_acc, dim3((n + 255) / 256), dim3(256), 0, st, col_acc, ncol, pair_acc, npair, rare_dev);
+  hipLaunchKernelGGL(dq_init_acc, dim3((n + 255) / 256), dim3(256), 0, st, col_acc, ncol, pair_acc, npair, rare_dev,
+                     win, win ? nwin : 0);
   return hipGetLastError();
 }
 
-}
+hipError_t launch_window_finish(const ColTask* tasks, int32_t ntasks, const IntWin* win, const uint32_t* win_bits,
+                                uint32_t* hll_acc, hipStream_t st) {
+  if (ntasks == 0 || !win) return hipSuccess;
+  hipLaunchKernelGGL(dq_window_finish, dim3((uint32_t)ntasks), dim3(kBlock), 0, st, tasks, ntasks, win, win_bits, hll_acc);
+  return hipGetLastError();
+}
+
+}
diff --git a/deequ_amd/csrc/dq_numeric_loop.inc b/deequ_amd/csrc/dq_numeric_loop.inc
--- /dev/null
+++ b/deequ_amd/csrc/dq_numeric_loop.inc
@@ -0,0 +1,43 @@
+  for (int32_t rb = 0; rb < nr; rb += kRowsPerIter) {
+    const int64_t base = row0 + rb + wave * 512;
+    const int32_t rem = nr - rb - wave * 512;
+    const bool full = rb + kRowsPerIter <= nr;
+    uint64_t bits[8], m[8];
+    double x[8];
+    const int32_t vo = (rb + wave * 512 + lane) * (int32_t)sizeof(T);
+#pragma unroll
+    for (int j = 0; j < 8; ++j) {
+      if constexpr (sizeof(T) == 8) {
+        const auto w2 = __builtin_amdgcn_raw_buffer_load_b64(vr, vo + j * 512, 0, 2 );
+        bits[j] = ((uint64_t)w2[1] << 32) | w2[0];
+        if (KIND == CK_F64) x[j] = __builtin_bit_cast(double, bits[j]);
+        else x[j] = __builtin_fma((double)(int32_t)w2[1], 4294967296.0, (double)w2[0]);
+      } else if constexpr (KIND == CK_F32) {
+        const uint32_t w = __builtin_amdgcn_raw_buffer_load_b32(vr, vo + j * 256, 0, 2 );
+        bits[j] = w;
+        x[j] = (double)__builtin_bit_cast(float, w);
+      } else {
+        int32_t w;
+        if constexpr (sizeof(T) == 4) w = (int32_t)__builtin_amdgcn_raw_buffer_load_b32(vr, vo + j * 256, 0, 2 );
+        else if constexpr (sizeof(T) == 2) w = (int16_t)__builtin_amdgcn_raw_buffer_load_b16(vr, vo + j * 128, 0, 2 );
+        else w = (int8_t)__builtin_amdgcn_raw_buffer_load_b8(vr, vo + j * 64, 0, 2 );
+        bits[j] = (uint64_t)(int64_t)w;
+        x[j] = (double)w;
+      }
+    }
+    block_masks(validity, mask, base, rem, full, m);
+    uint64_t nf_any = 0;
+    if constexpr (ck_float(KIND) && !kLazy) {
+#pragma unroll
+      for (int j = 0; j < 8; ++j) nf_any |= __builtin_amdgcn_ballot_w64(!__builtin_isfinite(x[j])) & m[j];
+    }
+    if (ck_float(KIND) && !kLazy && nf_any != 0) {
+      float_block_checked<KIND, STATS, HLL>(vr, validity, mask, base, rem, vo, shift, s, a, regs, cnt_w, nan_v, pinf_v,
+                                            ninf_v);
+    } else {
+#pragma unroll
+      for (int j = 0; j < 8; ++j) cnt_w += __builtin_popcountll(m[j]);
+      if constexpr (DQ_NUMERIC_LOOP_WIN) numeric_block_win<KIND, STATS>(x, bits, m, shift, s, a, regs, wbits, (uint64_t)win_base, vr, vo, out_w);
+      else numeric_block<KIND, STATS, HLL>(x, bits, m, shift, s, a, regs, qmin);
+    }
+  }
diff --git a/deequ_amd/csrc/dq_plan.cpp b/deequ_amd/csrc/dq_plan.cpp
--- a/deequ_amd/csrc/dq_plan.cpp
+++ b/deequ_amd/csrc/dq_plan.cpp
@@ -44,7 +44,8 @@
                             bool has_regex);
 hipError_t launch_column_scan(int32_t variant, const ColTask* tasks, int32_t ntasks, int32_t part_base,
                               const ScanCols& cols, const ScanBitmaps& bm, int64_t n_rows, int64_t rows_per_range,
-                              int32_t nranges, ColPartial* partials, uint32_t* hll_acc, bool long_str, hipStream_t st);
+                              int32_t nranges, ColPartial* partials, uint32_t* hll_acc, const ScanWindows& sw, bool long_str,
+                              hipStream_t st);
 hipError_t launch_pair_scan(const PairWG* wgs, int32_t nwg, const ScanCols& cols, const ScanBitmaps& bm,
                             const uint32_t* ones, int64_t n_rows, int64_t rows_per_range, int32_t nranges,
                             CorrPartial* pair_part, ColPartial* col_part, int32_t* redo, bool all_f64, bool ring,
@@ -53,8 +54,12 @@
 hipError_t launch_finalize(int32_t ncol, int32_t nranges_col, const ColPartial* col_part, ColPartial* col_acc,
                            int32_t npair, int32_t nranges_pair, const CorrPartial* pair_part, CorrPartial* pair_acc,
                            int32_t has_pred, int32_t nranges_pred, const PredPartial* pred_part, PredPartial* pred_acc, const FinRanges& fr, int64_t* rare_dev, int64_t* rare_host,
+                           const ColTask* tasks, IntWin* win,
                            hipStream_t st);
+hipError_t launch_window_finish(const ColTask* tasks, int32_t ntasks, const IntWin* win, const uint32_t* win_bits,
+                                uint32_t* hll_acc, hipStream_t st);
 hipError_t launch_init_acc(ColPartial* col_acc, int32_t ncol, CorrPartial* pair_acc, int32_t npair, int64_t* rare_dev,
+                           IntWin* win, int32_t nwin,
                            hipStream_t st);
 
 static thread_local char g_err[1024] = "";
@@ -622,6 +627,10 @@
   int64_t* d_rare = nullptr;
   std::vector<uint8_t> str_long;
   int32_t str_path = 0;
+  IntWin* d_win = nullptr;
+  uint32_t* d_win_bits = nullptr;
+  int32_t n_win = 0;
+  std::vector<int32_t> win_task;
   int64_t prev_rows = 0;
   size_t h_stage_bytes = 0;
   PredProgram* d_prog = nullptr;
@@ -700,7 +709,7 @@
   p->ev_pool.clear();
   void* ptrs[] = {p->d_col_tasks, p->d_pair_tasks, p->d_pair_wgs, p->d_prog, p->d_col_part, p->d_pair_part,
                   p->d_pred_part, p->d_col_acc, p->d_hll_acc, p->d_pair_acc, p->d_pred_acc, p->d_regex, p->d_pair_redo,
-                  p->d_rare_dev};
+                  p->d_rare_dev, p->d_win, p->d_win_bits};
   for (void* q : ptrs)
     if (q) (void)hipFree(q);
   for (int i = 0; i < kMaxWhere; ++i)
@@ -716,7 +725,8 @@
 
 static dq_status reset_acc(dq_plan* p) {
   HIP_TRY(launch_init_acc(p->d_col_acc, (int32_t)p->col_tasks.size(), p->d_pair_acc, (int32_t)p->pair_tasks.size(),
-                          p->d_rare_dev, p->stream));
+                          p->d_rare_dev, p->d_win, p->n_win, p->stream));
+  if (p->d_win_bits) HIP_TRY(hipMemsetAsync(p->d_win_bits, 0, (size_t)p->n_win * kWinWords * sizeof(uint32_t), p->stream));
   if (p->n_hll) HIP_TRY(hipMemsetAsync(p->d_hll_acc, 0, (size_t)p->n_hll * kHllCopies * 512 * sizeof(uint32_t), p->stream));
   if (p->has_pred) HIP_TRY(hipMemsetAsync(p->d_pred_acc, 0, kPredAccCopies * sizeof(PredPartial), p->stream));
   if (p->total_rows > 0) p->prev_rows = p->total_rows;
@@ -1267,6 +1277,35 @@
   }
   (void)hipGetLastError();
   if (dq_status s = dmalloc(&p->d_hll_acc, (size_t)p->n_hll * kHllCopies * 512 * sizeof(uint32_t))) return s;
+  {
+    const char* e = std::getenv("DQ_INT_WINDOW");
+    const bool use = !(e && std::strcmp(e, "off") == 0);
+    std::vector<IntWin> wins;
+    for (size_t t = 0; t < nct; ++t) {
+      ColTask& ct = p->col_tasks[t];
+      ct.win = -1;
+      const int32_t v = ct.variant;
+      const bool narrow = v == CV_I16_SH || v == CV_I16_H || v == CV_I8_SH || v == CV_I8_H;
+      const bool wide = v == CV_I64_SH || v == CV_I64_H || v == CV_I32_SH || v == CV_I32_H;
+      if (!use || ct.hll_slot < 0 || !(narrow || wide)) continue;
+      IntWin w{};
+      w.mode = narrow ? WIN_STATIC : WIN_AUTO;
+      w.on = narrow ? 1 : 0;
+      w.base = v == CV_I16_SH || v == CV_I16_H ? INT16_MIN : narrow ? INT8_MIN : 0;
+      w.vmin = INT64_MAX;
+      w.vmax = INT64_MIN;
+      ct.win = (int32_t)wins.size();
+      wins.push_back(w);
+      p->win_task.push_back((int32_t)t);
+    }
+    p->n_win = (int32_t)wins.size();
+    if (p->n_win) {
+      if (dq_status s = dmalloc(&p->d_win, wins.size() * sizeof(IntWin))) return s;
+      if (dq_status s = dmalloc(&p->d_win_bits, wins.size() * kWinWords * sizeof(uint32_t))) return s;
+      HIP_TRY(hipMemcpyAsync(p->d_win, wins.data(), wins.size() * sizeof(IntWin), hipMemcpyHostToDevice, p->stream));
+      HIP_TRY(hipStreamSynchronize(p->stream));
+    }
+  }
   if (dq_status s = dmalloc(&p->d_pair_acc, npt * sizeof(CorrPartial))) return s;
   if (dq_status s = dmalloc(&p->d_pred_acc, kPredAccCopies * sizeof(PredPartial))) return s;
   if (nct) HIP_TRY(hipMemcpyAsync(p->d_col_tasks, p->col_tasks.data(), nct * sizeof(ColTask), hipMemcpyHostToDevice, p->stream));
@@ -1680,6 +1719,7 @@
   ScanBitmaps bm{};
   for (int b = 0; b < kMaxWhere; ++b) bm.where_bits[b] = p->d_where_bits[b];
   bm.rare_rows = p->d_rare_dev;
+  const ScanWindows sw{p->d_win, p->d_win_bits};
   if ((!p->pair_wgs.empty() || p->pred_jit) && words + 1 > p->ones_cap_words) {
     HIP_TRY(hipStreamSynchronize(p->stream));
     if (p->d_ones) (void)hipFree(p->d_ones);
@@ -1818,7 +1858,7 @@
     const auto& g = groups[gi];
     if (dq_status s = timed(p, 16 + g.variant, p->stream, [&] {
           return launch_column_scan(g.variant, p->d_col_tasks + g.first, g.count, g.first, sc, bm, n_rows,
-                                    vr[gi].first, vr[gi].second, p->d_col_part, p->d_hll_acc, str_long_of(g),
+                                    vr[gi].first, vr[gi].second, p->d_col_part, p->d_hll_acc, sw, str_long_of(g),
                                     p->stream);
         }))
       return s;
@@ -1836,7 +1876,7 @@
         return launch_finalize((int32_t)p->col_tasks.size(), nr_col, p->d_col_part, p->d_col_acc,
                                (int32_t)p->pair_tasks.size(), nr_pair, p->d_pair_part, p->d_pair_acc,
                                0 , nr_pred, p->d_pred_part, p->d_pred_acc,
-                               fr, p->d_rare_dev, p->d_rare, p->stream);
+                               fr, p->d_rare_dev, p->d_rare, p->d_col_tasks, p->d_win, p->stream);
       }))
     return s;
   p->total_rows += n_rows;
@@ -1880,6 +1920,9 @@
   void* const dst_hll = hs ? (void*)(hs + o_hll) : (void*)hll.data();
   void* const dst_pair = hs ? (void*)(hs + o_pair) : (void*)pair.data();
   void* const dst_pred = hs ? (void*)(hs + o_pred) : (void*)pred_copies.data();
+  if (p->n_win)
+    HIP_TRY(launch_window_finish(p->d_col_tasks, (int32_t)p->col_tasks.size(), p->d_win, p->d_win_bits, p->d_hll_acc,
+                                 p->stream));
   if (b_col) HIP_TRY(hipMemcpyAsync(dst_col, p->d_col_acc, b_col, hipMemcpyDeviceToHost, p->stream));
   if (b_hll) HIP_TRY(hipMemcpyAsync(dst_hll, p->d_hll_acc, b_hll, hipMemcpyDeviceToHost, p->stream));
   if (b_pair) HIP_TRY(hipMemcpyAsync(dst_pair, p->d_pair_acc, b_pair, hipMemcpyDeviceToHost, p->stream));
@@ -2124,6 +2167,45 @@
 }
 int32_t dq_plan_num_launches(const dq_plan* p) { return p ? p->launches_per_scan : 0; }
 
+int32_t dq_plan_int_window_count(const dq_plan* p) {
+  if (!p) return 0;
+  int32_t n = p->n_win;
+  for (const dq_plan* q : p->parts) n += dq_plan_int_window_count(q);
+  return n;
+}
+
+dq_status dq_plan_int_window(dq_plan* p, int32_t index, dq_int_window* out) {
+  if (!p) return set_error(DQ_E_INVALID, "dq_plan_int_window: plan is NULL");
+  if (!out) return set_error(DQ_E_INVALID, "dq_plan_int_window: out is NULL");
+  if (index < 0 || index >= dq_plan_int_window_count(p))
+    return set_error(DQ_E_INVALID, "dq_plan_int_window: index %d out of range (the plan has %d windows)", index,
+                     dq_plan_int_window_count(p));
+  for (size_t k = 0; k < p->parts.size(); ++k) {
+    const int32_t n = dq_plan_int_window_count(p->parts[k]);
+    if (index < n) {
+      if (dq_status s = dq_plan_int_window(p->parts[k], index, out)) return s;
+      out->column = p->part_cols[k][out->column];
+      return DQ_OK;
+    }
+    index -= n;
+  }
+  HIP_TRY(hipSetDevice(p->device));
+  IntWin w{};
+  HIP_TRY(hipMemcpyAsync(&w, p->d_win + index, sizeof(IntWin), hipMemcpyDeviceToHost, p->stream));
+  HIP_TRY(hipStreamSynchronize(p->stream));
+  const ColTask& ct = p->col_tasks[p->win_task[index]];
+  std::memset(out, 0, sizeof(*out));
+  out->column = ct.col;
+  out->has_where = ct.where >= 0;
+  out->on = w.on;
+  out->off_for_run = w.off_for_run;
+  out->is_static = w.mode == WIN_STATIC;
+  out->base = w.base;
+  out->rows_in = (int64_t)w.rows_in;
+  out->rows_out = (int64_t)w.rows_out;
+  return DQ_OK;
+}
+
 dq_status dq_plan_create_time(const dq_plan* p, double* total_ms, double* pred_jit_ms) {
   if (!p) return set_error(DQ_E_INVALID, "dq_plan_create_time: plan is NULL");
   if (total_ms) *total_ms = p->create_ms;
diff --git a/deequ_amd/runner.py b/deequ_amd/runner.py
--- a/deequ_amd/runner.py
+++ b/deequ_amd/runner.py
@@ -82,8 +82,18 @@
         L.check(L.lib.dq_plan_kernel_time(self.handle, kernel, ctypes.byref(ms), ctypes.byref(n)))
         return ms.value, n.value
 
+    def int_windows(self) -> List[dict]:
+        out = []
+        for i in range(L.lib.dq_plan_int_window_count(self.handle)):
+            w = L.IntWindow()
+            L.check(L.lib.dq_plan_int_window(self.handle, i, ctypes.byref(w)))
+            out.append({"column": self.columns[w.column], "has_where": bool(w.has_where), "on": bool(w.on),
+                        "off_for_run": bool(w.off_for_run), "is_static": bool(w.is_static), "base": w.base,
+                        "rows_in": w.rows_in, "rows_out": w.rows_out})
+        return out
+
     def scan(self, table: Table) -> None:
-        views = (L.ColumnView * max(1, len(self.columns)))()
+        views =(L.ColumnView * max(1, len(self.columns)))()
         for i, name in enumerate(self.columns):
             views[i] = table.columns[name].view()
         L.check(L.lib.dq_scan(self.handle, views, table.num_rows, self.chunk))
diff --git a/include/dqscan.h b/include/dqscan.h
--- a/include/dqscan.h
+++ b/include/dqscan.h
@@ -211,6 +211,19 @@
 void dq_plan_destroy(dq_plan* plan);
 int64_t dq_plan_bytes_per_row_x1000(const dq_plan* plan);
 int32_t dq_plan_num_launches(const dq_plan* plan);
+typedef struct dq_int_window {
+  int32_t column;
+  int32_t has_where;
+  int32_t on;
+  int32_t off_for_run;
+  int32_t is_static;
+  int32_t reserved;
+  int64_t base;
+  int64_t rows_in;
+  int64_t rows_out;
+} dq_int_window;
+int32_t dq_plan_int_window_count(const dq_plan* plan);
+dq_status dq_plan_int_window(dq_plan* plan, int32_t index, dq_int_window* out);
 dq_status dq_plan_enable_timing(dq_plan* plan, int32_t on);
 dq_status dq_plan_kernel_time(dq_plan* plan, int32_t kernel, double* total_ms, int64_t* launches);
 int64_t dq_plan_variant_bytes_per_row_x1000(const dq_plan* plan, int32_t variant);
```

Measured after the change: 30.49 billion rows/s, median of 6. No clear change (+0.3%).
